# SahakyanLab/GenomeAssembler_dev

Hardware: AMD Instinct MI355X
Metric: k-mers built+scored/sec (higher is better)
Workload: dtype u64 keys / u32 counts / f64 scores; 1 GPU; cfg2 (configs[2]): 100 x 50000 bp segments per GPU, 150 bp reads at 50x, k=31, build + breakage scoring of all contigs; mode=segments, segments_total=100, distinct_kmers_rank0=3843627, parallelism=segments sharded over 1 GPU(s), no collective

## Files before the change

### genomeassembler_dev_amd/_lib.py

```python
import ctypes as C
import os

_HERE = os.path.dirname(os.path.abspath(__file__))
LIB_PATH = os.environ.get("GASM_LIBGASM") or os.path.join(_HERE, "libgasm.so")

GASM_OK = 0
STATUS = {0: "GASM_OK", -1: "GASM_ERR_INVALID", -2: "GASM_ERR_NON_ACGT", -3: "GASM_ERR_NO_DEVICE", -4: "GASM_ERR_HIP",
          -5: "GASM_ERR_CAPACITY", -6: "GASM_ERR_RANGE", -7: "GASM_ERR_STATE", -8: "GASM_ERR_INTERNAL"}
TABLE_ROWS = 69904
MAX_TIP_ROUNDS = 8
MAX_BUBBLE_ROUNDS = 8
MAX_BUBBLE_LEN = 65535
MAX_COV_ROUNDS = 8
CORRECT_FIELDS = ("no_kmer", "clean", "corrected", "partial", "left", "bases_changed")
CORRECT_MAX_KMERS = 4096
THREAD_MAX_KMERS = 4096
MAX_SPAN_LEN = 65535
MAX_INSERT = 65535
PAIR_FIELDS = ("skipped", "none_placed", "one_placed", "same_contig", "reversed", "diff_contig")
MAP_MAX_MISMATCH = 255
MAP_MAX_BLOCKS = 8
MAP_FIELDS = ("short", "skipped", "unseeded", "rejected", "mapped_one", "mapped_multi", "blocks_dropped")
MAP_MAX_GAP = 16
MAPG_FIELDS = MAP_FIELDS + ("gapped",)
# ... 19 lines not shown
_PP = C.POINTER(C.c_void_p)


class BuildParams(C.Structure):
    _fields_ = [("size", _u32), ("k", _i32), ("genome_len_hint", _u64), ("min_count", _u32), ("strands", _u32), ("tip_len", _u32),
                ("tip_rounds", _u32), ("bubble_len", _u32), ("bubble_rounds", _u32), ("cov_cutoff", _u32), ("cov_len", _u32), ("cov_rounds", _u32)]

    @classmethod
    def make(cls, k, **fields):
        p = cls(size=C.sizeof(cls), k=int(k))
        for name, v in fields.items():
            setattr(p, name, int(v))
        return p


SYMBOLS = {
    "gasm_last_error": (C.c_char_p, []),
    "gasm_version": (C.c_char_p, []),
    "gasm_ctx_create": (_int, [_int, _PP]),
    "gasm_ctx_destroy": (None, [_vp]),
    "gasm_ctx_sync": (_int, [_vp]),
    "gasm_ctx_stream": (_vp, [_vp]),
    "gasm_get_contigs": (_int, [_vp, _vp, _u64, _int, _int, _int, _PP]),
    "gasm_get_contigs_from_reads": (_int, [_vp, _vp, _vp, _u64, _int, _int, _int, _PP]),
    "gasm_get_contigs_from_reads_solid": (_int, [_vp, _vp, _vp, _u64, _int, _int, _int, _u32, _PP]),
    "gasm_get_contigs_from_reads_strands": (_int, [_vp, _vp, _vp, _u64, _int, _int, _int, _u32, _u32, _PP]),
    "gasm_get_contigs_from_reads_tips": (_int, [_vp, _vp, _vp, _u64, _int, _int, _int, _u32, _u32, _u32, _u32, _PP]),
    "gasm_get_contigs_from_reads_bubbles": (_int, [_vp, _vp, _vp, _u64, _int, _int, _int, _u32, _u32, _u32, _u32, _u32, _u32, _PP]),
    "gasm_get_contigs_from_reads_params": (_int, [_vp, _vp, _vp, _u64, _int, _int, C.POINTER(BuildParams), _PP]),
    "gasm_contigs_count": (_u64, [_vp]),
    "gasm_contigs_data": (_vp, [_vp]),
    "gasm_contigs_offsets": (_vp, [_vp]),
    "gasm_contigs_rows": (_u64, [_vp]),
    "gasm_contigs_perm": (_vp, [_vp]),
    "gasm_contigs_distinct_count": (_u64, [_vp]),
    "gasm_contigs_key_words": (_int, [_vp]),
    "gasm_contigs_distinct_keys": (_vp, [_vp]),
    "gasm_contigs_distinct_mult": (_vp, [_vp]),
    "gasm_contigs_free": (None, [_vp]),
    "gasm_assemble_contigs": (_int, [_vp, _vp, _vp, _u64, _vp, _u64, _u64, _int, _PP]),
    "gasm_assemble_contigs_velvet": (_int, [_vp, _vp, _vp, _u64, _int, _int, _int, _PP]),
    "gasm_assemble_contigs_dev": (_int, [_vp, _vp, _vp, _u64, _vp, _u64, _u64, _int, _PP]),
    "gasm_assemble_contigs_velvet_dev": (_int, [_vp, _vp, _vp, _u64, _int, _int, _int, _PP]),
    "gasm_scaffolds_count": (_u64, [_vp]),
    "gasm_scaffolds_offsets": (_vp, [_vp]),
    "gasm_scaffolds_merge_device": (_int, [_vp, C.POINTER(_u64)]),
    "gasm_scaffolds_fetch": (_int, [_vp, _PP]),
    "gasm_scaffolds_free": (None, [_vp]),
    "gasm_calc_breakscore_dev": (_int, [_vp, _vp, _vp, _vp, _u64, _vp, _u64, _int, _vp, _vp, _u64, _vp, _int, _int, _PP]),
    "gasm_strlist_count": (_u64, [_vp]),
    "gasm_strlist_data": (_vp, [_vp]),
    "gasm_strlist_offsets": (_vp, [_vp]),
    "gasm_strlist_free": (None, [_vp]),
    "gasm_calc_breakscore": (_int, [_vp, _vp, _vp, _u64, _vp, _vp, _u64, _vp, _u64, _int, _vp, _vp, _u64, _vp, _int, _int,
                                    _PP]),
    "gasm_calc_breakscore_tables": (_int, [_vp, _vp, _vp, _u64, _vp, _vp, _u64, _vp, _u64, _int, _vp, _vp, _u64, _vp, _u32, _int, _int, _PP]),
    "gasm_calc_breakscore_tables_dev": (_int, [_vp, _vp, _vp, _vp, _u64, _vp, _u64, _int, _vp, _vp, _u64, _vp, _u32, _int, _int, _PP]),
    "gasm_batch_score_tables": (_int, [_vp, _int, _vp, _u32]),
    "gasm_batch_fetch_scores_table": (_int, [_vp, _u32, _PP, _PP, _PP, _PP, _PP]),
    "gasm_batch_fetch_score_fixed_table": (_int, [_vp, _u32, _PP, C.POINTER(_int)]),
    "gasm_scores_count": (_u64, [_vp]),
    "gasm_scores_sequence_len": (_vp, [_vp]),
    "gasm_scores_bp_score": (_vp, [_vp]),
    "gasm_scores_norm_by_break_freqs": (_vp, [_vp]),
    "gasm_scores_norm_by_len": (_vp, [_vp]),
    "gasm_scores_kmer_breaks": (_vp, [_vp]),
    "gasm_scores_lev_dist": (_vp, [_vp]),
    "gasm_scores_path_freq": (_vp, [_vp]),
    "gasm_scores_startpos": (_vp, [_vp]),
    "gasm_scores_prob_dist": (_vp, [_vp]),
    "gasm_scores_prob_dist_offsets": (_vp, [_vp]),
    "gasm_scores_ks": (_vp, [_vp]),
    "gasm_scores_lev_device": (_int, [_vp]),
    "gasm_coverage_percent": (_int, [_vp, _vp, _vp, _u64, C.c_int64, _vp]),
    "gasm_scores_free": (None, [_vp]),
    "gasm_levenshtein": (_int, [_vp, _u64, _vp, _u64, _int, C.POINTER(_i32)]),
    "gasm_batch_create": (_int, [_vp, _vp, _vp, _u64, _u32, _vp, _u32, _PP]),
    "gasm_batch_create_packed": (_int, [_vp, _vp, _vp, _u64, _u32, _vp, _u32, _PP]),
    "gasm_batch_from_files": (_int, [_vp, _vp, _u32, _int, _PP, C.POINTER(_u64)]),
    "gasm_batch_guided": (_int, [_vp]),
    "gasm_batch_fetch_guided": (_int, [_vp, _PP, _PP, _PP, _PP, _PP, _PP]),
    "gasm_batch_fetch_score_fixed": (_int, [_vp, _PP, C.POINTER(_int)]),
    "gasm_batch_build_plan": (_int, [_vp, C.POINTER(_i32), _int]),
    "gasm_batch_simulate": (_int, [_vp, _vp, _vp, _u32, _u32, C.c_double, _u64, _int, _vp, _PP]),
    "gasm_batch_fetch_read_starts": (_int, [_vp, _PP, _PP]),
    "gasm_read_files": (_int, [_vp, _u32, _int, _PP]),
    "gasm_read_files_device": (_int, [_vp, _vp, _u32, _int, _PP]),
    "gasm_packed_parsed_on_device": (_int, [_vp, _u32]),
    "gasm_packed_n_reads": (_u64, [_vp]),
    "gasm_packed_n_segments": (_u32, [_vp]),
    "gasm_packed_words": (_vp, [_vp]),
    "gasm_packed_read_off": (_vp, [_vp]),
    "gasm_packed_seg_read_off": (_vp, [_vp]),
    "gasm_packed_dropped": (_u64, [_vp]),
    "gasm_packed_free": (None, [_vp]),
    "gasm_batch_free": (None, [_vp]),
    "gasm_batch_build": (_int, [_vp, _int, _u64]),
    "gasm_batch_score": (_int, [_vp, _int, _vp]),
    "gasm_batch_build_solid": (_int, [_vp, _int, _u64, _u32]),
    "gasm_batch_build_strands": (_int, [_vp, _int, _u64, _u32, _u32]),
    "gasm_batch_strands": (_u32, [_vp]),
    "gasm_batch_build_tips": (_int, [_vp, _int, _u64, _u32, _u32, _u32, _u32]),
    "gasm_batch_tip_len": (_u32, [_vp]),
    "gasm_batch_tip_rounds": (_u32, [_vp]),
    "gasm_batch_fetch_tip_stats": (_int, [_vp, _PP, _PP]),
    "gasm_batch_build_bubbles": (_int, [_vp, _int, _u64, _u32, _u32, _u32, _u32, _u32, _u32]),
    "gasm_batch_bubble_len": (_u32, [_vp]),
    "gasm_batch_bubble_rounds": (_u32, [_vp]),
    "gasm_batch_fetch_bubble_stats": (_int, [_vp, _PP, _PP]),
    "gasm_batch_build_params": (_int, [_vp, C.POINTER(BuildParams)]),
    "gasm_batch_cov_cutoff": (_u32, [_vp]),
    "gasm_batch_cov_len": (_u32, [_vp]),
    "gasm_batch_cov_rounds": (_u32, [_vp]),
    "gasm_batch_fetch_lowcov_stats": (_int, [_vp, _PP, _PP]),
    "gasm_batch_contig_coverage": (_int, [_vp]),
    "gasm_batch_fetch_contig_coverage": (_int, [_vp, _PP, _PP]),
    "gasm_batch_fetch_contig_twins": (_int, [_vp, _PP]),
    "gasm_batch_contig_links": (_int, [_vp, _u32]),
    "gasm_batch_fetch_contig_links": (_int, [_vp, _PP, _PP, _PP, _PP, _PP]),
    "gasm_batch_place_pairs": (_int, [_vp, _u32]),
    "gasm_batch_fetch_pair_places": (_int, [_vp, _PP, _PP, _PP, C.POINTER(_u32)]),
    "gasm_batch_map_reads": (_int, [_vp, _u32]),
    "gasm_batch_fetch_read_map": (_int, [_vp, _PP, _PP, _PP, _PP]),
    "gasm_batch_map_reads_gapped": (_int, [_vp, _u32, _u32]),
    "gasm_batch_fetch_read_map_gapped": (_int, [_vp, _PP, _PP, _PP, _PP, _PP, _PP]),
    "gasm_batch_map_reads_gapped_ends": (_int, [_vp, _u32, _u32, _u32]),
    "gasm_batch_fetch_read_map_ends": (_int, [_vp, _PP, _PP]),
    "gasm_batch_map_reads_aligned": (_int, [_vp, _u32, _u32, _u32]),
    "gasm_batch_fetch_read_alignments": (_int, [_vp, _PP, _PP, C.POINTER(_u32)]),
    "gasm_batch_score_mapped": (_int, [_vp, _int, _int, _vp, _u32, _u32]),
    "gasm_batch_fetch_mapped_scores": (_int, [_vp, _u32, _PP, _PP, _PP, _PP, _PP, _PP, C.POINTER(_int)]),
    "gasm_batch_fetch_mapped_starts": (_int, [_vp, _PP, _PP]),
    "gasm_batch_fetch_solid_stats": (_int, [_vp, _PP, _PP]),
    "gasm_batch_kmer_spectrum": (_int, [_vp]),
    "gasm_batch_fetch_kmer_spectrum": (_int, [_vp, _PP]),
    "gasm_batch_correct_reads": (_int, [_vp, _PP]),
    "gasm_batch_fetch_correct_stats": (_int, [_vp, _PP]),
    "gasm_batch_fetch_reads": (_int, [_vp, _PP, _PP]),
    "gasm_batch_total_kmers": (_u64, [_vp]),
    "gasm_batch_total_reads": (_u64, [_vp]),
    "gasm_batch_fetch_distinct": (_int, [_vp, _PP, _PP, _PP, C.POINTER(_int)]),
    "gasm_batch_fetch_contigs": (_int, [_vp, _PP, _PP, _PP]),
    "gasm_batch_fetch_graph": (_int, [_vp, _PP, _PP]),
    "gasm_batch_fetch_scores": (_int, [_vp, _PP, _PP, _PP, _PP, _PP]),
    "gasm_batch_count_read_kmers": (_int, [_vp]),
    "gasm_batch_fetch_read_kmer_counts": (_int, [_vp, _PP]),
    "gasm_count_read_kmers": (_int, [_vp, _vp, _vp, _u64, _int, _vp, _vp, _u64, _vp]),
    "gasm_pool_create": (_int, [_vp, _vp, _u64, _u32, _vp, _u32, _PP]),
    "gasm_pool_free": (None, [_vp]),
    "gasm_pool_key_words": (_int, [_vp]),
    "gasm_pool_local_runs": (_int, [_vp, _int, _int, _PP]),
    "gasm_pool_pack_runs": (_int, [_vp, _vp, _u64, _vp, _vp]),
    "gasm_pool_merge_runs": (_int, [_vp, _u32, _u32, _vp, _vp, _vp, _vp, _PP]),
    "gasm_pool_fetch_fine_directory": (_int, [_vp, _PP, C.POINTER(_int)]),
    "gasm_pool_graph": (_int, [_vp, _u32]),
    "gasm_pool_piece_words": (_int, [_vp, _u32, _u32, _vp]),
    "gasm_pool_pack_reads": (_int, [_vp, _u32, _u32, _vp]),
    "gasm_pool_set_reads": (_int, [_vp, _vp, _u64, _u32, _vp, _vp, _vp]),
    "gasm_pool_score": (_int, [_vp, _int, _vp]),
    "gasm_pool_fetch_distinct": (_int, [_vp, _PP, _PP, _PP, C.POINTER(_int)]),
    "gasm_pool_fetch_contigs": (_int, [_vp, _PP, _PP, _PP]),
    "gasm_pool_fetch_scores": (_int, [_vp, _PP, _PP, _PP, _PP, _PP]),
    "gasm_comm_unique_id": (_int, [_vp]),
    "gasm_comm_create": (_int, [_vp, _vp, _int, _int, _PP]),
    "gasm_comm_create_virtual": (_int, [_vp, _int, _PP]),
    "gasm_comm_destroy": (None, [_vp]),
# ... 117 lines not shown
```

### genomeassembler_dev_amd/batch.py

```python
import ctypes as C
from fractions import Fraction

import numpy as np

from . import qtable, readkmers
from ._lib import CORRECT_FIELDS, MAP_FIELDS, MAP_MAX_GAP, MAP_MAX_MISMATCH, MAP_MAX_PIECES, MAPEND_FIELDS, MAPG_FIELDS, MAPSCORE_FIELDS, MAPSCORE_PARTIAL, MAPSCORE_SOURCES, MAX_TABLES, MAX_BUBBLE_ROUNDS, MAX_COV_ROUNDS, MAX_INSERT, MAX_SPAN_LEN, MAX_TIP_ROUNDS, PAIR_FIELDS, PLAN_FIELDS, BuildParams, check, default_context, lib
from .api import _check_build_opts, unpack_kmers
from .links import ContigLinks
from .pairs import PairPlaces
from .readmap import AlignedReadMap, GappedReadMap, MappedScores, ReadMap


def _arr(p, ctype, n):
    return np.ctypeslib.as_array(C.cast(p, C.POINTER(ctype)), shape=(n,)).copy() if n else np.zeros(0, ctype)


def weighted_median_half(mult_sum, n_edges):
    ms, ns = [int(x) for x in mult_sum], [int(x) for x in n_edges]
    order = sorted(range(len(ns)), key=lambda i: Fraction(ms[i], ns[i]))
    total, run = sum(ns), 0
    for i in order:
        run += ns[i]
        if 2 * run >= total:
            return ms[i] // (2 * ns[i])
# ... 233 lines not shown
            check(lib().gasm_batch_fetch_read_map_ends(self.h, *[C.byref(p) for p in pe]))
            ends = dict(end_gap=end_gap, rec_end=_arr(pe[0], C.c_int32, 4 * self.n_reads), end_counters=_arr(pe[1], C.c_uint64, self.n_segments * len(MAPEND_FIELDS)))
        return GappedReadMap(self.k, strands, max_edits, max_gap, contigs, rec, gap, pile, gpile, hist, cnt,
                             [t.tolist() for t in self.contig_twins()] if strands == 2 else None, getattr(self, "_seg_read_off", None), **ends)

    def align_reads(self, max_edits=6, max_gap=3, end_gap=3):
        if not 0 <= int(max_edits) <= MAP_MAX_MISMATCH:
            raise ValueError(f"max_edits must be 0..{MAP_MAX_MISMATCH}")
        if not 0 <= int(max_gap) <= MAP_MAX_GAP:
            raise ValueError(f"max_gap must be 0..{MAP_MAX_GAP}")
        if not 0 <= int(end_gap) <= MAP_MAX_GAP:
            raise ValueError(f"end_gap must be 0..{MAP_MAX_GAP}")
        max_edits, max_gap, end_gap = int(max_edits), int(max_gap), int(end_gap)
        check(lib().gasm_batch_map_reads_aligned(self.h, max_edits, max_gap, end_gap))
        ps, pe, pa, cols = [C.c_void_p() for _ in range(6)], [C.c_void_p() for _ in range(2)], [C.c_void_p() for _ in range(2)], C.c_uint32()
        check(lib().gasm_batch_fetch_read_map_gapped(self.h, *[C.byref(p) for p in ps]))
        check(lib().gasm_batch_fetch_read_map_ends(self.h, *[C.byref(p) for p in pe]))
        check(lib().gasm_batch_fetch_read_alignments(self.h, *[C.byref(p) for p in pa], C.byref(cols)))
        seg, o, contigs = self._contigs_by_segment()
        total = int(o[-1]) if int(seg[-1]) else 0
        W = int(cols.value)
        rec, gap = _arr(ps[0], C.c_int32, 4 * self.n_reads), _arr(ps[1], C.c_int32, 4 * self.n_reads)
        pile, gpile = _arr(ps[2], C.c_uint32, 4 * total), _arr(ps[3], C.c_uint32, 2 * total)
        hist, cnt = _arr(ps[4], C.c_uint32, self.n_segments * (max_edits + 1)), _arr(ps[5], C.c_uint64, self.n_segments * len(MAPG_FIELDS))
        strands = self.strands()
        return AlignedReadMap(self.k, strands, max_edits, max_gap, end_gap, contigs, rec, gap, pile, gpile, hist, cnt,
                              _arr(pe[0], C.c_int32, 4 * self.n_reads), _arr(pe[1], C.c_uint64, self.n_segments * len(MAPEND_FIELDS)),
                              _arr(pa[0], C.c_int32, 2 * MAP_MAX_PIECES * self.n_reads), _arr(pa[1], C.c_uint32, 4 * W * total), W,
                              self._read_lengths(), [t.tolist() for t in self.contig_twins()] if strands == 2 else None,
                              getattr(self, "_seg_read_off", None))

    def score_mapped(self, kmer=8, tables=None, source="gapped", partial=False):
        t = np.ascontiguousarray(qtable.load_normalised() if tables is None else tables, dtype=np.float64)
        if t.ndim == 1:
            t = t.reshape(1, -1)
        if t.ndim != 2 or t.shape[1] != qtable.ROWS:
            raise ValueError(f"tables must be rows of {qtable.ROWS} probabilities")
        if not 1 <= t.shape[0] <= MAX_TABLES:
            raise ValueError(f"tables must hold 1..{MAX_TABLES} rows")
        if source not in MAPSCORE_SOURCES:
            raise ValueError(f"source must be one of {sorted(MAPSCORE_SOURCES)}")
        if int(kmer) < 0:
            raise ValueError("kmer must be >= 0")
        T = int(t.shape[0])
        check(lib().gasm_batch_score_mapped(self.h, MAPSCORE_SOURCES[source], int(kmer), t.ctypes.data_as(C.c_void_p), T, MAPSCORE_PARTIAL if partial else 0))
        seg, o, contigs = self._contigs_by_segment()
        n = int(seg[-1])
        total = int(o[-1]) if n else 0
        per_table = []
        for i in range(T):
            ps, sh = [C.c_void_p() for _ in range(6)], C.c_int()
            check(lib().gasm_batch_fetch_mapped_scores(self.h, i, *[C.byref(p) for p in ps], C.byref(sh)))
            per_table.append((dict(bp_score=_arr(ps[0], C.c_double, n), bp_score_norm_by_break_freqs=_arr(ps[1], C.c_double, n),
                                   bp_score_norm_by_len=_arr(ps[2], C.c_double, n), kmer_breaks=_arr(ps[3], C.c_int32, n),
                                   sequence_len=_arr(ps[4], C.c_int32, n), seg_contig_off=seg), _arr(ps[5], C.c_int64, n), sh.value))
        sp, cp = C.c_void_p(), C.c_void_p()
        check(lib().gasm_batch_fetch_mapped_starts(self.h, C.byref(sp), C.byref(cp)))
        return MappedScores(int(kmer), source, bool(partial), contigs, per_table, _arr(sp, C.c_uint32, total),
                            _arr(cp, C.c_uint64, self.n_segments * len(MAPSCORE_FIELDS)))

    def suggest_cov_cutoff(self, segment):
        floor = getattr(self, "_min_count", 1) + 1
        ms, ns = self.contig_coverage(segment)
        if not len(ns):
            return floor
        return max(floor, weighted_median_half(ms, ns))

    def kmer_spectrum(self):
        check(lib().gasm_batch_kmer_spectrum(self.h))
        p = C.c_void_p()
        check(lib().gasm_batch_fetch_kmer_spectrum(self.h, C.byref(p)))
        n = self.n_segments * 256
        return np.ctypeslib.as_array(C.cast(p, C.POINTER(C.c_uint64)), shape=(n,)).copy().reshape(self.n_segments, 256)

    def build_plan(self):
        rows = lib().gasm_batch_build_plan(self.h, None, 0)
        if rows < 0:
            check(rows)
        out = (C.c_int32 * (rows * len(PLAN_FIELDS)))()
        check(min(0, lib().gasm_batch_build_plan(self.h, out, len(out))))
        blocks = [dict(zip(PLAN_FIELDS, out[j * len(PLAN_FIELDS):(j + 1) * len(PLAN_FIELDS)])) for j in range(rows)]
        return dict(blocks[0], blocks=blocks)

    def score(self, kmer=8, table=None):
        t = np.ascontiguousarray(qtable.load_normalised() if table is None else table, dtype=np.float64)
        if t.size != qtable.ROWS:
            raise ValueError(f"table must hold {qtable.ROWS} probabilities")
        self._table = t
        check(lib().gasm_batch_score(self.h, int(kmer), t.ctypes.data_as(C.c_void_p)))
        return self

    def score_tables(self, kmer, tables):
        t = np.ascontiguousarray(tables, dtype=np.float64)
        if t.ndim != 2 or t.shape[1] != qtable.ROWS:
            raise ValueError(f"tables must be rows of {qtable.ROWS} probabilities")
        self._table = t[0] if len(t) else None
        check(lib().gasm_batch_score_tables(self.h, int(kmer), t.ctypes.data_as(C.c_void_p), t.shape[0]))
        return self

    def count_read_kmers(self):
        check(lib().gasm_batch_count_read_kmers(self.h))
        p = C.c_void_p()
        check(lib().gasm_batch_fetch_read_kmer_counts(self.h, C.byref(p)))
        n = self.n_segments * qtable.ROWS
        a = np.ctypeslib.as_array(C.cast(p, C.POINTER(C.c_uint32)), shape=(n,)).copy() if n else np.zeros(0, np.uint32)
        self._rkc = a.reshape(self.n_segments, qtable.ROWS)
        return self._rkc

    def read_kmer_counts(self, segment, kmer):
        if getattr(self, "_rkc", None) is None:
            self.count_read_kmers()
        return self._rkc[segment, readkmers.table_slice(kmer)]

    def correct_reads(self):
        h = C.c_void_p()
        check(lib().gasm_batch_correct_reads(self.h, C.byref(h)))
        new = SegmentBatch.__new__(SegmentBatch)
        new.ctx, new.h, new.k, new._table = self.ctx, h, None, None
        new.n_segments, new.n_reads = self.n_segments, int(lib().gasm_batch_total_reads(h))
        return new

    def correction_stats(self, as_dict=False):
        p = C.c_void_p()
        check(lib().gasm_batch_fetch_correct_stats(self.h, C.byref(p)))
        n = self.n_segments * len(CORRECT_FIELDS)
        a = np.ctypeslib.as_array(C.cast(p, C.POINTER(C.c_uint32)), shape=(n,)).copy().reshape(self.n_segments, len(CORRECT_FIELDS))
        return {name: a[:, i] for i, name in enumerate(CORRECT_FIELDS)} if as_dict else a

    def reads(self):
        d, o = C.c_void_p(), C.c_void_p()
        check(lib().gasm_batch_fetch_reads(self.h, C.byref(d), C.byref(o)))
        off = np.ctypeslib.as_array(C.cast(o, C.POINTER(C.c_uint64)), shape=(self.n_reads + 1,)).copy()
        total = int(off[-1])
        data = np.frombuffer(C.string_at(d, total), dtype=np.uint8).copy() if total else np.zeros(0, np.uint8)
        return data, off

    def read_strings(self):
        data, off = self.reads()
        raw = data.tobytes()
        return [raw[int(off[i]):int(off[i + 1])].decode() for i in range(self.n_reads)]

    def total_kmers(self):
        return int(lib().gasm_batch_total_kmers(self.h))

    def distinct(self):
        so, ks, ms, w = C.c_void_p(), C.c_void_p(), C.c_void_p(), C.c_int()
        check(lib().gasm_batch_fetch_distinct(self.h, C.byref(so), C.byref(ks), C.byref(ms), C.byref(w)))
        seg = np.ctypeslib.as_array(C.cast(so, C.POINTER(C.c_uint64)), shape=(self.n_segments + 1,)).copy()
        n = int(seg[-1])
        keys = np.ctypeslib.as_array(C.cast(ks, C.POINTER(C.c_uint64)), shape=(n * w.value,)).copy() if n else np.zeros(0, np.uint64)
        mult = np.ctypeslib.as_array(C.cast(ms, C.POINTER(C.c_uint32)), shape=(n,)).copy() if n else np.zeros(0, np.uint32)
        return seg, keys, mult, w.value

    def distinct_kmers(self, segment):
        seg, keys, mult, w = self.distinct()
        a, b = int(seg[segment]), int(seg[segment + 1])
        return unpack_kmers(keys[a * w:b * w], self.k, w), mult[a:b]

    def graph(self):
        seg = self.distinct()[0]
        n = int(seg[-1])
        fl, nx = C.c_void_p(), C.c_void_p()
        check(lib().gasm_batch_fetch_graph(self.h, C.byref(fl), C.byref(nx)))
        if not n:
            return np.zeros(0, np.uint8), np.zeros(0, np.uint32)
        return (np.ctypeslib.as_array(C.cast(fl, C.POINTER(C.c_uint8)), shape=(n,)).copy(),
# ... 74 lines not shown
```

### genomeassembler_dev_amd/csrc/capi.hip

```cpp
#include <algorithm>
#include <atomic>
#include <functional>
#include <memory>
#include <mutex>
#include <new>
#include <thread>

#include "pipeline.h"
#include "scaffolds.h"

struct gasm_strlist {
    std::vector<char> data;
    std::vector<u64> off;
};

struct gasm_contigs {
    std::vector<char> data;
    std::vector<u64> off;
    u64 rows = 0;
    std::vector<u32> perm;
    int words = 1;
    std::vector<u64> dkeys;
    std::vector<u32> dmult;
};
// ... 1166 lines not shown
    return GASM_OK;
}

int gasm_batch_score(gasm_batch* b, int kmer, const double* table) {
    API_GUARD_BEGIN
    return batch_score(b, "gasm_batch_score", kmer, table, 1);
    API_GUARD_END
}

int gasm_batch_score_tables(gasm_batch* b, int kmer, const double* tables, uint32_t n_tables) {
    API_GUARD_BEGIN
    return batch_score(b, "gasm_batch_score_tables", kmer, tables, n_tables);
    API_GUARD_END
}

int gasm_batch_guided(gasm_batch* b) {
    API_GUARD_BEGIN
    if (!b) { gasm_set_error("batch is null"); return GASM_ERR_INVALID; }
    if (!b->built || !b->scored) { gasm_set_error("gasm_batch_guided needs gasm_batch_build and gasm_batch_score first"); return GASM_ERR_STATE; }
    GCHK(batch_finish(b));
    StepSlot& x = b->S();
    GCHK(pipeline_score_fetch(x.cx, x.ss));
    return guided_build(x.cx, b->rd, x.bs, x.dp, x.ss, b->tb[0], b->score_kmer, b->guided);
    API_GUARD_END
}

int gasm_batch_fetch_guided(gasm_batch* b, const uint64_t** seg_off, const uint64_t** off, const char** data, const double** bp_score,
                            const double** norm_by_len, const int32_t** kmer_breaks) {
    API_GUARD_BEGIN
    if (!b || !seg_off || !off || !data || !bp_score || !norm_by_len || !kmer_breaks) { gasm_set_error("null argument"); return GASM_ERR_INVALID; }
    if (!b->guided.valid) { gasm_set_error("fetch before gasm_batch_guided"); return GASM_ERR_STATE; }
    GuidedState& g = b->guided;
    GCHK(guided_fetch_text(b->S().cx, g));
    *seg_off = g.h_seg_off.data(); *off = g.h_text_off.data(); *data = g.h_text.data();
    *bp_score = g.ss.h_bp.data(); *norm_by_len = g.ss.h_nl.data(); *kmer_breaks = g.ss.h_breaks.data();
    return GASM_OK;
    API_GUARD_END
}

static int batch_fetch_fixed(gasm_batch* b, uint32_t t, const int64_t** fx, int* shift) {
    if (!b || !fx || !shift) { gasm_set_error("null argument"); return GASM_ERR_INVALID; }
    if (!b->scored) { gasm_set_error("gasm_batch_fetch_score_fixed needs a scored batch"); return GASM_ERR_STATE; }
    if (t >= b->score_tables) { gasm_set_error("table %u of a score with %u table(s)", t, b->score_tables); return GASM_ERR_INVALID; }
    GCHK(batch_finish(b));
    StepSlot& x = b->S();
    if (!x.ss.graph) {
        gasm_set_error("the batch was scored in FP64, not in fixed point (reads shorter than k, or a table with NaN / infinite entries or a "
                       "range the 64-bit fixed point cannot hold): there are no fixed-point sums");
        return GASM_ERR_STATE;
    }
    const u32 P = x.bs.n_contigs;
    b->h_fx.resize(P);
    const size_t fx_off = (x.ss.stride * 4 + 15) & ~(size_t)15;
    HIPCHK(hipSetDevice(b->ctx->device));
    if (P) HIPCHK(hipMemcpyAsync(b->h_fx.data(), static_cast<const char*>(x.ss.d_total.p) + fx_off + (size_t)t * x.ss.stride * 8, (size_t)P * 8, hipMemcpyDeviceToHost, x.cx->stream));
    HIPCHK(hipStreamSynchronize(x.cx->stream));
    *fx = b->h_fx.data();
    *shift = b->tb[t].fix_shift;
    return GASM_OK;
}

int gasm_batch_fetch_score_fixed(gasm_batch* b, const int64_t** fx, int* shift) {
    API_GUARD_BEGIN
    return batch_fetch_fixed(b, 0, fx, shift);
    API_GUARD_END
}

int gasm_batch_fetch_score_fixed_table(gasm_batch* b, uint32_t t, const int64_t** fx, int* shift) {
    API_GUARD_BEGIN
    return batch_fetch_fixed(b, t, fx, shift);
    API_GUARD_END
}

int gasm_batch_build_plan(gasm_batch* b, int32_t* out, int n) {
    API_GUARD_BEGIN
    if (!b || n < 0 || (n > 0 && !out)) { gasm_set_error("gasm_batch_build_plan: bad argument"); return GASM_ERR_INVALID; }
    if (!b->built) { gasm_set_error("gasm_batch_build_plan before gasm_batch_build"); return GASM_ERR_STATE; }
    GCHK(batch_finish(b));
    if (n >= GASM_PLAN_FIELDS) pipeline_build_plan(b->rd, b->S().bs, out);
    return 1;
    API_GUARD_END
}

int gasm_batch_count_read_kmers(gasm_batch* b) {
    API_GUARD_BEGIN
    if (!b) { gasm_set_error("batch is null"); return GASM_ERR_INVALID; }
    if (!b->rkc_checked) GCHK(read_kmer_windows_check(b->rd));
    b->rkc_checked = true;
    HIPCHK(hipSetDevice(b->ctx->device));
    GCHK(b->d_rkc.ensure((size_t)b->n_segments * GASM_TABLE_ROWS * 4));
    GCHK(launch_read_kmer_count(b->ctx, b->rd, b->d_rkc.as<u32>()));
    b->rkc_counted = true;
    return GASM_OK;
    API_GUARD_END
}

int gasm_batch_fetch_read_kmer_counts(gasm_batch* b, const uint32_t** counts) {
    API_GUARD_BEGIN
    if (!b || !counts) { gasm_set_error("gasm_batch_fetch_read_kmer_counts: null argument"); return GASM_ERR_INVALID; }
    if (!b->rkc_counted) { gasm_set_error("gasm_batch_fetch_read_kmer_counts before gasm_batch_count_read_kmers"); return GASM_ERR_STATE; }
    b->h_rkc.resize((size_t)b->n_segments * GASM_TABLE_ROWS);
    HIPCHK(hipSetDevice(b->ctx->device));
    HIPCHK(hipMemcpyAsync(b->h_rkc.data(), b->d_rkc.p, b->h_rkc.size() * 4, hipMemcpyDeviceToHost, b->ctx->stream));
    HIPCHK(hipStreamSynchronize(b->ctx->stream));
    *counts = b->h_rkc.data();
    return GASM_OK;
    API_GUARD_END
}

int gasm_batch_correct_reads(gasm_batch* b, gasm_batch** out) {
    API_GUARD_BEGIN
    if (!b || !out) { gasm_set_error("gasm_batch_correct_reads: null argument"); return GASM_ERR_INVALID; }
    *out = nullptr;
    if (!b->built) { gasm_set_error("gasm_batch_correct_reads before a build"); return GASM_ERR_STATE; }
    GCHK(batch_finish(b));
    StepSlot& x = b->S();
    DBuf words, stats;
    struct Rel { DBuf &a, &b; ~Rel() { a.release(); b.release(); } } rel{words, stats};
    GCHK(pipeline_correct_reads(x.cx, b->rd, x.bs, words, stats));
    HIPCHK(hipStreamSynchronize(x.cx->stream));
    const DevReads& rd = b->rd;
    return new_batch(b->ctx, b->n_segments, rd.n_reads, out, [&](gasm_batch* nb) {
        GCHK(nb->rd.adopt_packed(b->ctx, words, rd.fixed_len ? nullptr : rd.h_read_off.data(), rd.n_reads, rd.fixed_len, rd.h_seg_read_off.data(), rd.n_segments));
        std::swap(nb->d_correct, stats);
        nb->corrected = true;
        return (int)GASM_OK;
    });
    API_GUARD_END
}

int gasm_batch_fetch_correct_stats(gasm_batch* b, const uint32_t** stats) {
    API_GUARD_BEGIN
    if (!b || !stats) { gasm_set_error("gasm_batch_fetch_correct_stats: null argument"); return GASM_ERR_INVALID; }
    if (!b->corrected) { gasm_set_error("gasm_batch_fetch_correct_stats: not a batch made by gasm_batch_correct_reads"); return GASM_ERR_STATE; }
    b->h_correct.resize((size_t)b->n_segments * GASM_CORRECT_FIELDS);
    HIPCHK(hipSetDevice(b->ctx->device));
    HIPCHK(hipMemcpyAsync(b->h_correct.data(), b->d_correct.p, b->h_correct.size() * 4, hipMemcpyDeviceToHost, b->ctx->stream));
    HIPCHK(hipStreamSynchronize(b->ctx->stream));
    *stats = b->h_correct.data();
    return GASM_OK;
    API_GUARD_END
}

int gasm_batch_fetch_reads(gasm_batch* b, const char** ascii, const uint64_t** read_off) {
    API_GUARD_BEGIN
    if (!b || !ascii || !read_off) { gasm_set_error("gasm_batch_fetch_reads: null argument"); return GASM_ERR_INVALID; }
    GCHK(pipeline_fetch_reads(b->ctx, b->rd, b->h_reads_ascii, b->h_reads_off));
    *ascii = b->h_reads_ascii.data();
    *read_off = b->h_reads_off.data();
    return GASM_OK;
    API_GUARD_END
}

static const u32 kRkcRow[9] = {0, 0, 0, 0, 16, 0, 272, 0, 4368};

int gasm_count_read_kmers(gasm_ctx* ctx, const char* reads, const uint64_t* read_off, uint64_t n_reads, int kmer, const char* keys,
                          const uint64_t* key_off, uint64_t n_keys, uint32_t* counts) {
    API_GUARD_BEGIN
    if (!ctx || (n_reads && (!reads || !read_off)) || (keys && n_keys && !key_off)) { gasm_set_error("gasm_count_read_kmers: null argument"); return GASM_ERR_INVALID; }
    if (kmer != 2 && kmer != 4 && kmer != 6 && kmer != 8) { gasm_set_error("kmer must be 2, 4, 6 or 8 (got %d)", kmer); return GASM_ERR_INVALID; }
    const u64 n_out = keys ? n_keys : (1ull << (2 * kmer));
    if (n_out && !counts) { gasm_set_error("gasm_count_read_kmers: counts is null"); return GASM_ERR_INVALID; }
    std::vector<u32> row;
    if (keys) {
        row.resize(n_keys);
        for (u64 i = 0; i < n_keys; ++i) {
// ... 105 lines not shown
```

### genomeassembler_dev_amd/csrc/kernels.h

```cpp
#pragma once
#include <hip/hip_runtime.h>
#include <stdint.h>

#include <type_traits>

#include "device_utils.h"
#include "keyops.h"

struct ReadSet {
    const u64* words;
    const u64* read_off;
    const u64* seg_read_off;
    const u32* seg_tile_start;
    const uint4* tile_info;
    u32 fixed_len;
    u32 n_segments;
};

__device__ __forceinline__ void read_span(const ReadSet& rs, u64 r, u64* p0, u32* len) {
    if (rs.fixed_len) { *p0 = rs.read_off ? rs.read_off[r] : r * rs.fixed_len; *len = rs.fixed_len; }
    else { const u64 a = rs.read_off[r]; *p0 = a; *len = (u32)(rs.read_off[r + 1] - a); }
}

struct GraphView {
    const void* dk_key;
    const u32* dstart;
    const u16* fdir;
    int k;
    int bbits;
    int fbits;
};

template <class K>
__device__ __forceinline__ u32 graph_lower_bound(const GraphView& gv, u32 seg, const K& t, u32* bucket_hi) {
    const K* dk = reinterpret_cast<const K*>(gv.dk_key);
    const u32 nb = 1u << gv.bbits;
    const int low = 2 * gv.k - gv.bbits;
    const u32 gb = seg * nb + (gv.bbits ? kfield(t, low) : 0u);
    uint2 dd;
    __builtin_memcpy(&dd, gv.dstart + gb, 8);
    const u32 base = dd.x;
    *bucket_hi = dd.y;
    const int bshift = low > gv.fbits ? low - gv.fbits : 0;
    const u32 nbin = 1u << gv.fbits;
    const u16* f = gv.fdir + (u64)gb * (nbin + 1) + (kfield(t, bshift) & (nbin - 1));
    u32 ff;
    __builtin_memcpy(&ff, f, 4);
    u32 lo = base + (ff & 0xFFFFu);
    u32 hi = base + (ff >> 16);
    if (hi > *bucket_hi) hi = *bucket_hi;
    if (lo > hi) lo = hi;
    while (hi - lo > 4) {
        const u32 m = (lo + hi) >> 1;
        if (kless(dk[m], t)) lo = m + 1;
        else hi = m;
    }
    while (lo < hi && kless(dk[lo], t)) ++lo;
    return lo;
}

struct PathSet {
    const u64* words;
    const u64* p_off;
    const u32* seg_path_off;
    u32 n_segments;
};

#define GASM_KT 16
#define GASM_SCORE_PATH_CAP 6144
#define GASM_TBL 4096
#define GASM_TBL_LIMIT 2816
constexpr int dedup_bins(int tbl) { return tbl / 4; }
constexpr int dedup_fbits(int tbl) { return tbl <= 4 ? 0 : 1 + dedup_fbits(tbl / 2); }
static_assert(1 << dedup_fbits(2048) == dedup_bins(2048) && 1 << dedup_fbits(GASM_TBL) == dedup_bins(GASM_TBL), "the bins are a power of two");

enum : u32 {
    GASM_FLAG_OVERFLOW = 0,
    GASM_FLAG_RANK_FAILED = 1,
    GASM_FLAG_SCORE_MISMATCH = 2,
    GASM_FLAG_DEDUP_DONE = 8,
    GASM_FLAG_CONTIG_DONE = 9,
    GASM_FLAG_SOLID_DONE = 10,
    GASM_FLAG_ACTIVE = 16,
    GASM_FLAG_ACTIVE_N = 40,
    GASM_FLAG_WORDS = 64,
    GASM_FLAG_CURSORS = 64,
    GASM_FLAG_BYTES = 256,
    GASM_OVF_TABLE = 1,
    GASM_OVF_REGION = 2,
    GASM_OVF_TIP_RANK = 4,
};
static_assert(GASM_FLAG_ACTIVE + GASM_FLAG_ACTIVE_N <= GASM_FLAG_WORDS && GASM_FLAG_WORDS * 4 == GASM_FLAG_BYTES, "flag area layout");

template <class W>
struct BuildReport {
    W* w;
    u32 S;
    __host__ __device__ W& dstart(u32 s) const { return w[s]; }
    __host__ __device__ W& cstart(u32 s) const { return (w + S + 1)[s]; }
    __host__ __device__ W& bstart_lo(u32 s) const { return (w + 2 * S + 2)[2 * s]; }
    __host__ __device__ W& bstart_hi(u32 s) const { return (w + 2 * S + 2)[2 * s + 1]; }
    __host__ __device__ W& flags() const { return w[4 * S + 4]; }
    __host__ __device__ W& rank_failed() const { return w[4 * S + 5]; }
    __host__ __device__ W& ticket() const { return w[4 * S + 6]; }
    static size_t words(u32 S) { return 4 * (size_t)S + 8; }
};

__global__ void k_pack_ascii(const u8* ascii, u64 nbases_host, const u64* nbases_dev, u64* words, u32* err);
#define GASM_TILE_WG 512
template <class K> struct TileStage {
    static constexpr u32 KPU = 16 / sizeof(K);
    static constexpr u32 CAP = KeyTraits<K>::NFL * GASM_TILE_WG * KPU;
    static constexpr u32 TRASH = GASM_TILE_WG / 8;
    static constexpr u32 BYTES = (CAP + TRASH) * (u32)sizeof(K);
    static constexpr u32 PAD_ROOM = (KeyTraits<K>::NFL * KPU - KeyTraits<K>::KT) * GASM_TILE_WG;
};
template <class K> struct ScatterLds {
    u32 nb;
    static constexpr u32 n_key = TileStage<K>::CAP + TileStage<K>::TRASH;
    constexpr u32 n_comb() const { return (nb + 1) & ~1u; }
    constexpr u32 n_sub() const { return 4 * nb; }
    static constexpr u32 n_dummy = 4;
    static constexpr u32 n_tmp = 12;
    constexpr size_t total() const { return TileStage<K>::BYTES + (size_t)nb * 8 + ((size_t)n_sub() + n_dummy + n_tmp) * 4 + 32; }
};
template <class K> struct PartitionLds {
    u32 nb;
    static constexpr u32 n_key = TileStage<K>::CAP + TileStage<K>::TRASH;
    constexpr u32 n_comb() const { return nb; }
    constexpr u32 n_sub() const { return 4 * nb; }
    static constexpr u32 n_dummy = 4;
    static constexpr u32 n_tmp = 12;
    constexpr u32 n_cin() const { return nb; }
    constexpr size_t total() const { return TileStage<K>::BYTES + (size_t)n_comb() * 16 + (2 * ((size_t)n_sub() + n_dummy) + n_tmp + n_cin()) * 4; }
};
#define GASM_FLUSH_WGS 1024
#define GASM_FLUSH_SLOTS (GASM_FLUSH_WGS * (GASM_TILE_WG / 64))
__device__ __forceinline__ u32 flush_slot(u32 wave) { return (blockIdx.x % GASM_FLUSH_WGS) * (GASM_TILE_WG / 64) + wave; }
template <class K> __global__ void k_tile_hist(ReadSet rs, const uint4* tinfo, int k, int bbits, u32 g, u32 n_tiles, ushort4* tcnt);
__global__ void k_tile_scan(ReadSet rs, int bbits, u32 padm, const ushort4* tcnt, u32* toff, u32* hist, u32* flags);
template <class TO> __global__ void k_scan_excl(const u32* in, TO* out, u32 n);
__global__ void k_copy_u64(const u64* a, u64* b, u32 n);
template <class K>
__global__ void k_bucket_scatter(ReadSet rs, const uint4* tinfo, int k, int bbits, u32 g, u32 padm, u32 n_tiles, const u64* bstart, const u32* toff,
                                 const ushort4* tcnt, K* keys, u64 scratch);
#define GASM_RT_MAX 16
template <class K>
__global__ void k_bucket_partition(ReadSet rs, const uint4* tinfo, int k, int bbits, u32 g, u32 padm, u32 n_tiles, const u64* bstart, u32* cursor,
                                   K* keys, u64 scratch, u32* flags);
template <class K, int TBL>
__global__ void k_bucket_dedup(K* keys, u32* mult, const u64* bstart, const u32* blen, u32* bucket_d, u32* overflow, u16* fdir, int low_bits, u32* dstart);
#define GASM_BUCKET_MAX 65535
template <class K>
__global__ void k_bucket_dedup_multi(const K* keys, K* keys_out, u32* mult, const u64* bstart, u32* bucket_d, u32* overflow, u16* fdir, int low_bits);
template <class K>
__global__ void k_bucket_solid(K* keys, u32* mult, const u64* bstart, u32* bucket_d, u16* fdir, int low_bits, int fbits, int bbits, u32 min_count,
                               u32* removed, u32* done, u32* dstart);
template <class K>
__global__ void k_tip_mark(GraphView gv, u32 n_segments, u32 chunks, const u8* eflag, const u32* clen, const u32* nxt, const u32* dk_cnt, const u64* bstart,
                           u32* mult, u32 tip_len, u32* flags, u32* tips);
template <class K>
__global__ void k_bubble_mark(GraphView gv, u32 n_segments, u32 chunks, const u8* eflag, const u32* clen, const u32* nxt, const u32* dk_cnt, const u64* bstart,
                              u32* mult, u32 bubble_len, u32* flags, u32* bubbles);
__global__ void k_kmer_spectrum(const u32* dstart, u32 nb, const u32* dk_cnt, u32 n_segments, u32 chunks, u32* hist);
template <class K>
__global__ void k_lowcov_mark(GraphView gv, u32 n_segments, u32 chunks, const u8* eflag, const u32* clen, const u32* nxt, const u32* dk_cnt, const u64* bstart,
                              u32* mult, u32 cov_len, u32 cov_cutoff, u32* flags, u32* removed);
__global__ void k_contig_cov(const u32* dstart, u32 nb, u32 n_segments, u32 chunks, const u64* link, const u32* e_cid, const u32* dk_cnt,
                             const u32* seg_cstart, unsigned long long* msum, u32* nedges);
template <class K>
__global__ void k_bucket_gather(const K* keys, const u32* mult, const u64* bstart, const u32* dstart, K* dk_key, u32* dk_cnt, u32* claim, u8* eflag,
                                u32* flags);
template <class K> __global__ void k_edge_target(GraphView gv, u32 n_segments, u32 chunks, u32* tgt, u32* claim);
__global__ void k_edge_multi(GraphView gv, u32 n_segments, u32 chunks, const u32* tgt, const u32* claim, u8* eflag);
template <class K>
__global__ void k_node_flags(GraphView gv, u32 n_segments, u32 chunks, const u32* claim, u8* eflag, u64* link, u32* clen);
__global__ void k_edge_next(GraphView gv, u32 n_segments, u32 chunks, const u32* tgt, const u8* eflag, u32* nxt, u64* link);
__global__ void k_link_jump(GraphView gv, u32 n_segments, u32 chunks, u64* link, const u32* prev_active, u32* active, int jumps, const u32* nxt,
                            u32* clen);
__global__ void k_rank_rulers(GraphView gv, u32 n_segments, u32 chunks, u64* link, u32* rtab, u32 rshift, u32* flags);
__global__ void k_rank_lds(GraphView gv, const u32* rtab, u64* link, int max_rounds, u32 rshift, u32 lds_entries, u32* flags);
__global__ void k_chain_len(const u32* nxt, const u64* link, u32* clen, const u32* n_edges_p);
__global__ void k_contig_scan(GraphView gv, const u8* eflag, const u32* clen, u32* e_cid, u64* e_coff, u32* seg_ncontig,
                              u64* seg_cbases, u32* done, u32* seg_cstart, u64* seg_bstart, const u32* flags, u32* report, u32 ticket);
__global__ void k_contig_place(GraphView gv, const u8* eflag, const u32* seg_cstart, const u64* seg_bstart, u32* e_cid, u64* e_coff,
                               u64* c_off, u32 n_segments, u32 chunks);
template <class K>
__global__ void k_contig_emit(GraphView gv, const u64* link, const u32* nxt, const u64* e_coff, u8* out, u32 n_segments, u32 chunks);
__global__ void k_reads_both_strands(const u64* words, const u64* read_off, const u64* seg_read_off, u32 fixed_len, u32 n_segments, u64 n_reads, u32 g,
                                     unsigned long long* out);
template <class K>
__global__ void k_contig_twin(GraphView gv, const u64* link, const u32* e_cid, const u64* c_off, const u32* seg_cstart, const u8* text, u32 n_segments,
                              u32* twin, u32* bad);

template <class K>
__global__ void k_pack_runs(const K* keys, const u32* mult, const u64* bstart, const u32* bucket_d, const u32* gb_list, const u64* dst_off, K* out_keys,
                            u32* out_cnt);
template <class K, int TBL>
__global__ void k_bucket_merge(const K* in_keys, const u32* in_cnt, const u64* run_off, const u32* run_len, u32 n_src, K* out_keys, u32* out_cnt,
                               const u64* bstart, u32* bucket_d, u32* overflow, u16* fdir, int low_bits, const u64* src_base);
__global__ void k_repack_reads(const u64* src, const u64* dir, u64* words_out);
__global__ void k_piece_positions(const u64* piece_first, const u64* piece_word_off, u32 n_pieces, u64 n_reads, u32 fixed_len, u64* pos);
__global__ void k_slice_last(const u32* a, const u64* off, u32 n, u32* out);

__global__ void k_chain_expand(const u64* cwords, const u64* c_off, const u64* sig_off, const u32* elem_contig, const u32* elem_skip, const u64* elem_pos,
                               const u64* out_off, u32 n_scaffolds, u64* out, u64 n_words);
struct ChainSigs {
    const u64* sig_off;
    const u32* elem_contig;
    const u32* elem_skip;
    const u64* elem_pos;
};
__global__ void k_str_bitonic(const u64* words, const u64* off, u32* idx, u32 n_pow2, u32 kk, u32 j, ChainSigs cs);
__global__ void k_str_bitonic_block(const u64* words, const u64* off, u32* idx, u32 n_pow2, u32 kk, u32 j0, ChainSigs cs);
__global__ void k_str_adjacent_eq(const u64* words, const u64* off, const u32* idx, u32 n, u8* same_as_prev, ChainSigs cs);
__global__ void k_unpack_ascii(const u64* words, u64 nbases, u8* out);
__global__ void k_guided_chain(PathSet ps, const unsigned long long* fx, int k, u32* g_next, u32* g_prev, u32* dbg_order);
__global__ void k_asm_match(const u64* cwords, const u64* c_off, u32 n, int k, u8* match, u8* row_any, u8* level_any);
__global__ void k_asm_merge(const u32* perm, u32 rows, u32 n, int k, const u32* clen, const u8* match, const u8* row_any, const u8* level_any,
                            const u64* cwords, const u64* c_off, u32* out_next, u8* out_ov, u32* out_heads, u32* out_nchains, u8* need_host);

__global__ void k_sim_weights(const u64* gwords, const u64* gbase, const u64* woff, u32 n_segments, int kmer, const long long* fixw, u64* w);
template <class T> __global__ void k_seg_scan_incl(T* a, const u64* off);
__global__ void k_sim_draw(const u64* cum, const u64* woff, const u64* doff, const u64* glen, u64 seed, u32 read_len, u32* start, u32* keep);
__global__ void k_sim_compact(const u32* start, const u32* keep, const u32* rank, const u64* doff, const u64* seg_read_off, u32* kept_start);
__global__ void k_sim_extract(const u64* gwords, const u64* gbase, const u64* seg_read_off, const u32* kept_start, u32 read_len, unsigned long long* out);

template <int LS>
__global__ void k_read_kmer_count(const u64* words, const u64* read_off, const u64* seg_read_off, u32 fixed_len, u32 n_segments, u32* out);

struct ContigIndex {
    const u64* link;
// ... 106 lines not shown
```

### genomeassembler_dev_amd/csrc/kernels_build.hip

```cpp
#include "device_utils.h"
#include "keyops.h"
#include "kernels.h"
#include "dedup_order.h"

typedef unsigned long long u64x2 __attribute__((ext_vector_type(2)));

typedef unsigned int u32x4nt __attribute__((ext_vector_type(4)));
__device__ __forceinline__ uint4 stream_load16(const uint4* p) {
    const u32x4nt v = __builtin_nontemporal_load(reinterpret_cast<const u32x4nt*>(p));
    return make_uint4(v.x, v.y, v.z, v.w);
}
__device__ __forceinline__ void stream_store16(u64x2 v, u64x2* p) { __builtin_nontemporal_store(v, p); }

__global__ void __launch_bounds__(GASM_WG) k_pack_ascii(const u8* __restrict__ ascii, u64 nbases_host, const u64* __restrict__ nbases_dev,
                                                        u64* __restrict__ words, u32* __restrict__ err) {
    const u64 nbases = nbases_dev ? *nbases_dev : nbases_host;
    const u64 nwords = (nbases + 31) / 32 + 4;
    bool ok = true;
    for (u64 t = (u64)blockIdx.x * GASM_WG + threadIdx.x; t < nwords; t += (u64)gridDim.x * GASM_WG) {
        const u64 b0 = t << 5;
        u64 w = 0;
        if (b0 + 32 <= nbases) {
            const uint4* src = reinterpret_cast<const uint4*>(ascii + b0);
            const uint4 v0 = src[0], v1 = src[1];
// ... 231 lines not shown
            pf.bs_lo = b.x; pf.bs_hi = b.y;
        }
        tile_fetch<K>(rs, ti, g, k, pf.rl, pf.nv);
    };
    TileInfo ti = tile_decode(tinfo, tile);
    TilePrefetch<K> pf;
    fetch(tile, ti, pf);
    pf.template wait_all_but<0>();
    for (;;) {
        u32 total;
        if (one) {
            const u32 c0 = pf.c01 & 0xFFFFu, c1 = pf.c01 >> 16, c2 = pf.c23 & 0xFFFFu, c3 = pf.c23 >> 16;
            const u32 cnt = c0 + c1 + c2 + c3, padc = (cnt + padm) & ~padm;
            const u32 soff = block_excl_scan<GASM_TILE_WG>(padc, s_tmp, &total);
            if (tid < nb) {
                *reinterpret_cast<uint4*>(&s_cur[4 * tid]) = make_uint4(soff, soff + c0, soff + c0 + c1, soff + c0 + c1 + c2);
                s_comb[tid] = (((u64)pf.bs_hi << 32) | pf.bs_lo) + pf.toff - soff;
                for (u32 i = cnt; i < padc; ++i) s_key[soff + i] = key_filler<K>(tid, bshift);
            }
        } else {
            u32 carry = 0;
            for (u32 b0 = 0; b0 < nb; b0 += GASM_TILE_WG) {
                const u32 b = b0 + tid;
                const ushort4 c = tcnt[(u64)tile * nb + b];
                const u32 cnt = sub_total(c), padc = (cnt + padm) & ~padm;
                u32 tot;
                const u32 soff = carry + block_excl_scan<GASM_TILE_WG>(padc, s_tmp, &tot);
                *reinterpret_cast<uint4*>(&s_cur[4 * b]) = make_uint4(soff, soff + c.x, soff + c.x + c.y, soff + c.x + c.y + c.z);
                s_comb[b] = bstart[(u64)ti.seg * nb + b] + toff[(u64)tile * nb + b] - soff;
                for (u32 i = cnt; i < padc; ++i) s_key[soff + i] = key_filler<K>(b, bshift);
                carry += tot;
            }
            total = carry;
        }
        __syncthreads();
        const auto w = pf.rl.prep();
        const u32 nv = pf.nv;
        K key[KT];
        u32 idx[KT];
        static_for<KT>([&](auto J) {
            constexpr u32 j = J;
            key[j] = w.template key<j>(k);
            const u32 bkt = bbits ? w.template top_hi<j>() >> (32 - bbits) : 0u;
            idx[j] = atomicAdd(&s_cur[j < nv ? 4 * bkt + sub : 4 * nb], 1u);
        });
        const u32 tnext = tile + 1 < tile_end ? tile + 1 : tile;
        const TileInfo tin = tile_decode(tinfo, tnext);
        fetch(tnext, tin, pf);
        const u32 trash = CAP + wv * 8 + (ln & 7u);
#pragma unroll
        for (u32 j = 0; j < KT; ++j) s_key[j < nv ? idx[j] : trash] = key[j];
        __syncthreads();
        static_assert(NFL % 3 == 0, "flush passes come in threes");
#pragma unroll
        for (u32 u0 = 0; u0 < NFL; u0 += 3) {
            u64x2 w[3];
            u64 cb[3];
#pragma unroll
            for (u32 u = 0; u < 3; ++u) w[u] = *reinterpret_cast<const u64x2*>(s_key + (tid + GASM_TILE_WG * (u0 + u)) * KPU);
#pragma unroll
            for (u32 u = 0; u < 3; ++u) {
                u32 bkt = 0;
                if (bbits) {
                    if constexpr (KPU == 2) bkt = (u32)(w[u].x >> bshift) & (nb - 1);
                    else bkt = kfield(K128{w[u].x, w[u].y}, bshift) & (nb - 1);
                }
                cb[u] = s_comb[bkt];
            }
#pragma unroll
            for (u32 u = 0; u < 3; ++u) {
                const u32 i = (tid + GASM_TILE_WG * (u0 + u)) * KPU;
                stream_store16(w[u], reinterpret_cast<u64x2*>(keys + (i < total ? cb[u] + i : my_scratch)));
            }
        }
        if (++tile >= tile_end) break;
        __syncthreads();
        ti = tin;
        pf.template wait_all_but<NFL>();
    }
}
template __global__ void k_bucket_scatter<u64>(ReadSet, const uint4*, int, int, u32, u32, u32, const u64*, const u32*, const ushort4*, u64*, u64);
template __global__ void k_bucket_scatter<K128>(ReadSet, const uint4*, int, int, u32, u32, u32, const u64*, const u32*, const ushort4*, K128*, u64);

template <class K>
__global__ void __launch_bounds__(GASM_TILE_WG, 4) k_bucket_partition(ReadSet rs, const uint4* __restrict__ tinfo, int k, int bbits, u32 g, u32 padm,
                                                                    u32 n_tiles, const u64* __restrict__ bstart, u32* __restrict__ cursor,
                                                                    K* __restrict__ keys, u64 scratch, u32* __restrict__ flags) {
    extern __shared__ __align__(16) unsigned char s_raw[];
    constexpr u32 KT = KeyTraits<K>::KT;
    constexpr u32 NFL = KeyTraits<K>::NFL;
    constexpr u32 KPU = TileStage<K>::KPU;
    constexpr u32 CAP = TileStage<K>::CAP;
    const u32 nb = 1u << bbits;
    const u32 tid = threadIdx.x, wv = tid >> 6, ln = tid & 63, sub = tid & 3u;
    const PartitionLds<K> lds{nb};
    K* s_key = reinterpret_cast<K*>(s_raw);
    uint4* s_comb = reinterpret_cast<uint4*>(s_key + lds.n_key);
    u32* s_base = reinterpret_cast<u32*>(s_comb + lds.n_comb());
    u32* s_cnt = s_base + lds.n_sub() + lds.n_dummy;
    u32* s_tmp = s_cnt + lds.n_sub() + lds.n_dummy;
    u32* s_cin = s_tmp + lds.n_tmp;
    const int bshift = 2 * k - bbits;
    const bool carry = padm != 0;
    const u32 ush = carry ? (u32)__builtin_ctz(padm + 1) - (KPU == 2 ? 1u : 0u) : 0u;
    const u32 n_carry = carry ? nb << ush : 0u;
    const u32 unit_m = carry ? KPU - 1 : 0u;

    const u32 per_wg = (n_tiles + gridDim.x - 1) / gridDim.x;
    const u32 tile_end = min(n_tiles, (blockIdx.x + 1) * per_wg);
    u32 tile = blockIdx.x * per_wg;
    if (tile >= tile_end) return;
    for (u32 e = tid; e < 4 * nb + 4; e += GASM_TILE_WG) s_cnt[e] = 0;

    Roll<K> rl;
    u32 nv;
    auto fetch = [&](const TileInfo& t) { tile_fetch<K>(rs, t, g, k, rl, nv); };
    TileInfo ti = tile_decode(tinfo, tile);
    fetch(ti);
    rl.template wait_all_but<0>();
    __syncthreads();
    bool fresh = true;
    u64x2 cu = {0, 0};
    for (;;) {
        const auto w = rl.prep();
        const u32 nv_now = nv;
        const u32 seg = ti.seg;
        u32 idx[KT];
        static_for<KT>([&](auto J) {
            constexpr u32 j = J;
            const u32 bkt = bbits ? w.template top_hi<j>() >> (32 - bbits) : 0u;
            idx[j] = atomicAdd(&s_cnt[j < nv_now ? 4 * bkt + sub : 4 * nb], 1u);
        });
        const u32 tnext = tile + 1 < tile_end ? tile + 1 : tile;
        const TileInfo tin = tile_decode(tinfo, tnext);
        fetch(tin);
        const bool last = !carry || tile + 1 >= tile_end || tin.seg != seg;
        __syncthreads();
        u32 t = tid, zero = 0;
        __asm__ volatile("" : "+v"(t), "+v"(zero));
        u32 c0 = 0, c1 = 0, c2 = 0, c3 = 0, cin = 0;
        if (t < nb) {
            const uint4 c = *reinterpret_cast<const uint4*>(&s_cnt[4 * t]);
            c0 = c.x; c1 = c.y; c2 = c.z; c3 = c.w;
            if (!fresh) cin = s_comb[t].w & 31u;
        }
        const u32 cnt = cin + c0 + c1 + c2 + c3, flush = cnt & ~padm;
        const u32 res = last ? (cnt + padm) & ~padm : flush;
        u32 total;
        const u32 both = block_excl_scan_open<GASM_TILE_WG>((((cnt + padm) & ~padm) << 16) | ((cnt + unit_m) & ~unit_m), s_tmp, &total);
        const bool lines = (total >> 16) <= CAP;
        const u32 soff = lines ? both >> 16 : both & 0xFFFFu;
        u32 run = 0;
        u64 beg = 0, end = 0;
        if (t < nb) {
            const u32 gb = seg * nb + t;
            if (res) run = atomicAdd(&cursor[gb], res);
            beg = bstart[gb]; end = bstart[gb + 1];
            const u32 s0 = soff + cin;
            *reinterpret_cast<uint4*>(&s_base[4 * t]) = make_uint4(s0, s0 + c0, s0 + c0 + c1, s0 + c0 + c1 + c2);
            *reinterpret_cast<uint4*>(&s_cnt[4 * t]) = make_uint4(zero, zero, zero, zero);
            s_cin[t] = (soff << 5) | cin;
            s_comb[t].w = (lines ? 1u << 31 : 0u) | ((soff + flush) << 5) | (cnt - flush);
        }
        __syncthreads();
        if (t < n_carry) {
            const u32 b = t >> ush, f = (t & ((1u << ush) - 1u)) * KPU;
            if (!fresh) {
                const u32 v = s_cin[b], n = v & 31u;
                K* const dst = s_key + (v >> 5) + f;
                if constexpr (KPU == 2) {
                    if (f < n) dst[0] = cu.x;
                    if (f + 1 < n) dst[1] = cu.y;
                } else {
                    if (f < n) *reinterpret_cast<u64x2*>(dst) = cu;
                }
            }
            const u32 v = s_comb[b].w, n = v & 31u;
            if ((v >> 31) && n) {
                K* const dst = s_key + ((v << 1) >> 6) + f;
                if (f >= n) dst[0] = key_filler<K>(b, bshift);
                if constexpr (KPU == 2) if (f + 1 >= n) dst[1] = key_filler<K>(b, bshift);
            }
        }
        {
            static_for<KT>([&](auto J) {
                constexpr u32 j = J;
                const u32 bkt = bbits ? w.template top_hi<j>() >> (32 - bbits) : 0u;
                idx[j] += s_base[4 * bkt + sub];
            });
            const u32 trash = CAP + wv * 8 + (ln & 7u);
            static_for<KT>([&](auto J) {
                constexpr u32 j = J;
                s_key[j < nv_now ? idx[j] : trash] = w.template key<j>(k);
            });
        }
        if (t < nb) {
            const bool fits = (u64)run + res <= end - beg;
            const u64 cb = beg + run - soff;
            s_comb[t] = make_uint4((u32)cb, (u32)(cb >> 32), fits ? soff + flush : 1u << 31, (lines ? 1u << 31 : 0u) | ((soff + flush) << 5) | (cnt - flush));
            if (!fits) atomicOr(flags + GASM_FLAG_OVERFLOW, GASM_OVF_REGION);
        }
        __syncthreads();
        if (t < n_carry) {
            const u32 b = t >> ush, f = (t & ((1u << ush) - 1u)) * KPU;
            const uint4 c = s_comb[b];
            const u32 rbeg = (c.w << 1) >> 6, n = c.w & 31u;
            cu = *reinterpret_cast<const u64x2*>(s_key + rbeg + f);
            if (last && n && !(c.z >> 31)) {
                u64x2 o = cu;
                if constexpr (KPU == 2) {
                    const u64 fl = key_filler<u64>(b, bshift);
                    if (f >= n) o.x = fl;
                    if (f + 1 >= n) o.y = fl;
                } else if (f >= n) {
                    const K128 fl = key_filler<K128>(b, bshift);
                    o.x = fl.hi; o.y = fl.lo;
                }
                stream_store16(o, reinterpret_cast<u64x2*>(keys + ((((u64)c.y << 32) | c.x) + rbeg + f)));
            }
        }
        const u64 my_scratch = scratch + (u64)flush_slot(t >> 6) * KPU;
        static_assert(NFL % 3 == 0, "flush passes come in threes");
#pragma unroll
        for (u32 u0 = 0; u0 < NFL; u0 += 3) {
            u64x2 wd[3];
            uint4 cb[3];
#pragma unroll
            for (u32 u = 0; u < 3; ++u) wd[u] = *reinterpret_cast<const u64x2*>(s_key + (t + GASM_TILE_WG * (u0 + u)) * KPU);
#pragma unroll
            for (u32 u = 0; u < 3; ++u) {
                u32 bkt = 0;
                if (bbits) {
                    if constexpr (KPU == 2) bkt = (u32)(wd[u].x >> bshift) & (nb - 1);
                    else bkt = kfield(K128{wd[u].x, wd[u].y}, bshift) & (nb - 1);
                }
                cb[u] = s_comb[bkt];
            }
#pragma unroll
            for (u32 u = 0; u < 3; ++u) {
                const u32 i = (t + GASM_TILE_WG * (u0 + u)) * KPU;
                stream_store16(wd[u], reinterpret_cast<u64x2*>(keys + ((int)i < (int)cb[u].z ? (((u64)cb[u].y << 32) | cb[u].x) + i : my_scratch)));
            }
        }
        if (++tile >= tile_end) break;
        ti = tin;
        fresh = last;
        rl.template wait_all_but<NFL>();
    }
}
template __global__ void k_bucket_partition<u64>(ReadSet, const uint4*, int, int, u32, u32, u32, const u64*, u32*, u64*, u64, u32*);
template __global__ void k_bucket_partition<K128>(ReadSet, const uint4*, int, int, u32, u32, u32, const u64*, u32*, K128*, u64, u32*);

#define GASM_SLOT_LOCKED 0xFFFFFFFFu

__device__ __forceinline__ u64x2 lds_load128(const void* p) {
    __asm__ volatile("" ::: "memory");
    return *reinterpret_cast<const u64x2*>(p);
}
__device__ __forceinline__ uint4 lds_load128u(const void* p) {
    __asm__ volatile("" ::: "memory");
    return *reinterpret_cast<const uint4*>(p);
}

template <int TBL>
__device__ __forceinline__ bool dedup_step(u64* t_key, u32* t_cnt, u32* n_distinct, u64 key, u32& set) {
    constexpr u32 NSETS = TBL / 2;
    const u64x2 c = lds_load128(&t_key[2 * set]);
    int slot = c.x == key ? 0 : c.y == key ? 1 : -1;
    if (slot < 0) {
        const int emp = c.x == GASM_EMPTY64 ? 0 : c.y == GASM_EMPTY64 ? 1 : -1;
        if (emp < 0) { set = (set + 1) & (NSETS - 1); return false; }
        const u64 old = atomicCAS(reinterpret_cast<unsigned long long*>(&t_key[2 * set + emp]), (unsigned long long)GASM_EMPTY64,
                                  (unsigned long long)key);
        if (old == GASM_EMPTY64) atomicAdd(n_distinct, 1u);
        else if (old != key) return false;
        slot = emp;
    }
    atomicAdd(&t_cnt[2 * set + slot], 1u);
    return true;
}
template <int TBL>
__device__ __forceinline__ bool dedup_step(K128* t_key, u32* t_cnt, u32* n_distinct, const K128& key, u32& set) {
    constexpr u32 NSETS = TBL / 2;
    __asm__ volatile("" ::: "memory");
    const uint2 c = *reinterpret_cast<const uint2*>(&t_cnt[2 * set]);
    const u32 cc[2] = {c.x, c.y};
#pragma unroll
    for (int q = 0; q < 2; ++q) {
        if (cc[q] == GASM_SLOT_LOCKED) return false;
        if (cc[q] == 0) {
            if (atomicCAS(&t_cnt[2 * set + q], 0u, GASM_SLOT_LOCKED) != 0u) return false;
            t_key[2 * set + q] = key;
            __builtin_amdgcn_fence(__ATOMIC_RELEASE, "workgroup");
            __hip_atomic_store(&t_cnt[2 * set + q], 1u, __ATOMIC_RELAXED, __HIP_MEMORY_SCOPE_WORKGROUP);
            atomicAdd(n_distinct, 1u);
            return true;
        }
        const u64x2 kq = lds_load128(&t_key[2 * set + q]);
        if (kq.x == key.hi && kq.y == key.lo) { atomicAdd(&t_cnt[2 * set + q], 1u); return true; }
    }
    set = set + 1 >= NSETS - 1 ? 0u : set + 1;
    return false;
}

constexpr int GASM_DEDUP_NLD = 3, GASM_DEDUP_NLDW = 6, GASM_DEDUP_WGS = 6;
__device__ __forceinline__ void publish_u32(u32* p, u32 v) { __hip_atomic_store(p, v, __ATOMIC_RELAXED, __HIP_MEMORY_SCOPE_AGENT); }
__device__ __forceinline__ void publish_u64(u64* p, u64 v) { __hip_atomic_store(p, v, __ATOMIC_RELAXED, __HIP_MEMORY_SCOPE_AGENT); }
__device__ __forceinline__ bool count_in_last(u32* done) {
    __asm__ volatile("s_waitcnt vmcnt(0)" ::: "memory");
    return __hip_atomic_fetch_add(done, 1u, __ATOMIC_RELAXED, __HIP_MEMORY_SCOPE_AGENT) == gridDim.x - 1;
}

__device__ __forceinline__ void dedup_last_scan(const u32* __restrict__ bucket_d, u32* __restrict__ dstart, u32 n, u32* __restrict__ done, u32* s_word,
                                                u32* s_waves ) {
    if (!dstart) return;
    __syncthreads();
    if (threadIdx.x == 0) *s_word = count_in_last(done) ? 1u : 0u;
    __syncthreads();
    if (!*s_word) return;
    const u32 per = (n + GASM_WG - 1) / GASM_WG, a = min(n, threadIdx.x * per), b = min(n, a + per);
    u32 sum = 0;
    for (u32 i = a; i < b; ++i) sum += __hip_atomic_load(&bucket_d[i], __ATOMIC_RELAXED, __HIP_MEMORY_SCOPE_AGENT);
    const u32 inc = wave_incl_scan(sum);
    __syncthreads();
    if ((threadIdx.x & 63) == 63) s_waves[threadIdx.x >> 6] = inc;
    __syncthreads();
    u32 ex = inc - sum, tot = 0;
    for (u32 w = 0; w < GASM_WG / 64; ++w) { const u32 t = s_waves[w]; if (w < (threadIdx.x >> 6)) ex += t; tot += t; }
    for (u32 i = a; i < b; ++i) { dstart[i] = ex; ex += __hip_atomic_load(&bucket_d[i], __ATOMIC_RELAXED, __HIP_MEMORY_SCOPE_AGENT); }
    if (threadIdx.x == 0) dstart[n] = tot;
}

template <class K, int TBL>
__global__ void __launch_bounds__(GASM_WG, TBL == 4096 ? 3 : sizeof(K) == 8 ? GASM_DEDUP_WGS : 4)
k_bucket_dedup(K* __restrict__ keys, u32* __restrict__ mult, const u64* __restrict__ bstart, const u32* __restrict__ blen, u32* __restrict__ bucket_d,
               u32* __restrict__ overflow, u16* __restrict__ fdir, int low_bits, u32* __restrict__ dstart) {
    constexpr int LIMIT = TBL / 16 * 11;
    constexpr int BINS = dedup_bins(TBL);
    constexpr int LOG_TBL = TBL == 4096 ? 12 : 11;
    constexpr bool WIDE = sizeof(K) == 16;
    constexpr int LOG_SETS = LOG_TBL - 1;
    constexpr u32 NSETS = 1u << LOG_SETS;
    static_assert(TBL == 4096 || TBL == 2048, "table size");
    __shared__ __align__(32) K t_key[TBL];
    __shared__ __align__(16) u32 t_cnt[TBL];
    u32 *s_tmp, *w_distinct, *w_overflow;
    if constexpr (WIDE) {
        s_tmp = reinterpret_cast<u32*>(&t_key[TBL - 2]);
        w_distinct = &t_cnt[TBL - 2];
        w_overflow = &t_cnt[TBL - 1];
    } else {
        __shared__ u32 s_tmp_narrow[8];
        s_tmp = s_tmp_narrow;
        w_distinct = &s_tmp_narrow[4];
        w_overflow = &s_tmp_narrow[5];
    }
    static_assert((TBL - LIMIT) * sizeof(K) >= 2 * BINS * sizeof(u32), "the bins must fit behind the sorted entries");
    u32* const s_start = reinterpret_cast<u32*>(t_key + LIMIT);
    u32* const s_cur = s_start + BINS;
    const u32 bucket = blockIdx.x;
    const u64 beg = bstart[bucket], end = bstart[bucket + 1];
// ... 36 lines not shown
            u32 missed = 0, mfull = 0;
            {
                u32 set[KPL];
                u64x2 c[KPL];
#pragma unroll
                for (int q = 0; q < KPL; ++q) {
                    set[q] = khash(kx[q]) >> (32 - LOG_SETS);
                    c[q] = lds_load128(&t_key[2 * set[q]]);
                }
#pragma unroll
                for (int q = 0; q < KPL; ++q) {
                    const u64 key = kx[q];
                    if (kis_filler(key)) continue;
                    const int slot = c[q].x == key ? 0 : c[q].y == key ? 1 : -1;
                    if (slot >= 0) atomicAdd(&t_cnt[2 * set[q] + slot], 1u);
                    else {
                        missed |= 1u << q;
                        if (c[q].y != GASM_EMPTY64) mfull |= 1u << q;
                    }
                }
            }
            while (missed) {
                const u32 q = (u32)__builtin_ctz(missed);
                missed &= missed - 1;
                u64 key = kx[0];
#pragma unroll
                for (u32 e = 1; e < (u32)KPL; ++e) if (e == q) key = kx[e];
                u32 st = ((khash(key) >> (32 - LOG_SETS)) + (mfull >> q & 1u)) & (NSETS - 1);
                bool ok = false;
                for (u32 probe = 0; probe < 8 * NSETS && !ok; ++probe) ok = dedup_step<TBL>(t_key, t_cnt, w_distinct, key, st);
                if (!ok) *w_overflow = 1;
            }
        } else {
            u32 set[KPL];
            uint2 cn[KPL];
            u64x2 k0[KPL], k1[KPL];
#pragma unroll
            for (int q = 0; q < KPL; ++q) {
                set[q] = min(khash(kx[q]) >> (32 - LOG_SETS), NSETS - 2);
                __asm__ volatile("" ::: "memory");
                cn[q] = *reinterpret_cast<const uint2*>(&t_cnt[2 * set[q]]);
                k0[q] = lds_load128(&t_key[2 * set[q]]);
                k1[q] = lds_load128(&t_key[2 * set[q] + 1]);
            }
            u32 missed = 0;
#pragma unroll
            for (int q = 0; q < KPL; ++q) {
                const K128 key = kx[q];
                if (kis_filler(key)) continue;
                const bool r0 = cn[q].x != 0 && cn[q].x != GASM_SLOT_LOCKED, r1 = cn[q].y != 0 && cn[q].y != GASM_SLOT_LOCKED;
                if (r0 && k0[q].x == key.hi && k0[q].y == key.lo) atomicAdd(&t_cnt[2 * set[q]], 1u);
                else if (r0 && r1 && k1[q].x == key.hi && k1[q].y == key.lo) atomicAdd(&t_cnt[2 * set[q] + 1], 1u);
                else missed |= 1u << q;
            }
            while (missed) {
                const u32 q = (u32)__builtin_ctz(missed);
                missed &= missed - 1;
                K128 key = kx[0];
#pragma unroll
                for (u32 e = 1; e < (u32)KPL; ++e) if (e == q) key = kx[e];
                u32 st = min(khash(key) >> (32 - LOG_SETS), NSETS - 2);
                bool ok = false;
                for (u32 probe = 0; probe < 8 * NSETS && !ok; ++probe) ok = dedup_step<TBL>(t_key, t_cnt, w_distinct, key, st);
                if (!ok) *w_overflow = 1;
            }
        }
    }
    __syncthreads();
    if (*w_overflow || *w_distinct > (u32)LIMIT) {
        for (u32 i = threadIdx.x; i <= (u32)BINS; i += GASM_WG) fdir[(u64)bucket * (BINS + 1) + i] = 0;
        if (threadIdx.x == 0) { atomicOr(overflow + GASM_FLAG_OVERFLOW, GASM_OVF_TABLE); publish_u32(&bucket_d[bucket], 0u); }
        dedup_last_scan(bucket_d, dstart, gridDim.x, overflow + GASM_FLAG_DEDUP_DONE, s_tmp + 7, s_tmp);
        return;
    }
    const u32 d = *w_distinct;
    dedup_order<K, TBL, true>(t_key, t_cnt, s_start, s_cur, s_tmp, fdir, bucket, low_bits, d);
    for (u32 i = threadIdx.x; i < d; i += GASM_WG) { keys[beg + i] = t_key[i]; mult[beg + i] = t_cnt[i]; }
    if (threadIdx.x == 0) publish_u32(&bucket_d[bucket], d);
    dedup_last_scan(bucket_d, dstart, gridDim.x, overflow + GASM_FLAG_DEDUP_DONE, s_tmp + 7, s_tmp);
}
template __global__ void k_bucket_dedup<u64, 4096>(u64*, u32*, const u64*, const u32*, u32*, u32*, u16*, int, u32*);
template __global__ void k_bucket_dedup<u64, 2048>(u64*, u32*, const u64*, const u32*, u32*, u32*, u16*, int, u32*);
template __global__ void k_bucket_dedup<K128, 2048>(K128*, u32*, const u64*, const u32*, u32*, u32*, u16*, int, u32*);

template <class K>
__global__ void __launch_bounds__(GASM_WG) k_bucket_dedup_multi(const K* __restrict__ keys, K* __restrict__ keys_out, u32* __restrict__ mult,
                                                                const u64* __restrict__ bstart, u32* __restrict__ bucket_d,
                                                                u32* __restrict__ overflow, u16* __restrict__ fdir, int low_bits) {
    constexpr int TBL = 4096, LIMIT = TBL / 16 * 11, BINS = dedup_bins(TBL), LOG_SETS = 11, LOG_BINS = dedup_fbits(TBL);
    constexpr u32 NSETS = 1u << LOG_SETS;
    __shared__ __align__(32) K t_key[TBL];
    __shared__ __align__(16) u32 t_cnt[TBL];
    __shared__ u32 s_start[BINS];
    __shared__ u32 s_cur[BINS];
    __shared__ u32 s_tmp[8];
    const u32 bucket = blockIdx.x;
    const u64 beg = bstart[bucket], n = bstart[bucket + 1] - beg;
    const int bin_bits = low_bits < LOG_BINS ? low_bits : LOG_BINS;
    const int r_max = low_bits < 16 ? low_bits : 16;
    u16* const fd = fdir + (u64)bucket * (BINS + 1);
    auto give_up = [&]() {
        for (u32 i = threadIdx.x; i <= (u32)BINS; i += GASM_WG) fd[i] = 0;
        if (threadIdx.x == 0) { atomicOr(overflow + GASM_FLAG_OVERFLOW, GASM_OVF_TABLE); bucket_d[bucket] = 0; }
    };
    for (int r = 0;; ++r) {
        if (r > r_max) { give_up(); return; }
        const u32 npass = 1u << r;
        u32 total = 0;
        bool fits = true;
        for (u32 p = 0; p < npass; ++p) {
            for (u32 i = threadIdx.x; i < TBL; i += GASM_WG) { t_key[i] = key_empty<K>(); t_cnt[i] = 0; }
            for (u32 i = threadIdx.x; i < BINS; i += GASM_WG) s_start[i] = 0;
            if (threadIdx.x == 0) { s_tmp[4] = 0; s_tmp[5] = 0; s_tmp[6] = 0; }
            __syncthreads();
            for (u64 i = threadIdx.x; i < n; i += GASM_WG) {
                const K key = keys[beg + i];
                if (kis_filler(key)) continue;
                if (r && (kfield(key, low_bits - r) & (npass - 1)) != p) continue;
                if (__hip_atomic_load(&s_tmp[4], __ATOMIC_RELAXED, __HIP_MEMORY_SCOPE_WORKGROUP) > (u32)LIMIT) break;
                u32 st = khash(key) >> (32 - LOG_SETS);
                bool ok = false;
                for (u32 probe = 0; probe < 8 * NSETS && !ok; ++probe) ok = dedup_step<TBL>(t_key, t_cnt, &s_tmp[4], key, st);
                if (!ok) s_tmp[5] = 1;
            }
            __syncthreads();
            const u32 d = s_tmp[4];
            if (s_tmp[5] || d > (u32)LIMIT) { fits = false; break; }
            if (total + d > GASM_BUCKET_MAX) { give_up(); return; }
            u32 lo, hi;
            if (r <= bin_bits) { lo = p << (bin_bits - r); hi = (p + 1) << (bin_bits - r); }
            else { lo = p >> (r - bin_bits); hi = (p & ((1u << (r - bin_bits)) - 1u)) ? lo : lo + 1; }
            dedup_order<K, TBL, false, true>(t_key, t_cnt, s_start, s_cur, s_tmp, fdir, bucket, low_bits, d, total, lo, hi);
            for (u32 i = threadIdx.x; i < d; i += GASM_WG) { keys_out[beg + total + i] = t_key[i]; mult[beg + total + i] = t_cnt[i]; }
            total += d;
            __syncthreads();
        }
        if (!fits) { __syncthreads(); continue; }
        for (u32 i = (1u << bin_bits) + threadIdx.x; i <= (u32)BINS; i += GASM_WG) fd[i] = (u16)total;
        if (threadIdx.x == 0) bucket_d[bucket] = total;
        return;
    }
}
template __global__ void k_bucket_dedup_multi<u64>(const u64*, u64*, u32*, const u64*, u32*, u32*, u16*, int);
template __global__ void k_bucket_dedup_multi<K128>(const K128*, K128*, u32*, const u64*, u32*, u32*, u16*, int);

#define GASM_SOLID_ITEMS 4
template <class K>
__global__ void __launch_bounds__(GASM_WG) k_bucket_solid(K* __restrict__ keys, u32* __restrict__ mult, const u64* __restrict__ bstart,
                                                          u32* __restrict__ bucket_d, u16* __restrict__ fdir, int low_bits, int fbits, int bbits,
                                                          u32 min_count, u32* __restrict__ removed, u32* __restrict__ done, u32* __restrict__ dstart) {
    constexpr u32 MAX_BINS = dedup_bins(GASM_TBL);
    constexpr u32 CHUNK = GASM_WG * GASM_SOLID_ITEMS;
    __shared__ u32 s_bin[MAX_BINS];
    __shared__ u32 s_tmp[8];
    const u32 bucket = blockIdx.x;
    const u32 bins = 1u << fbits;
    const int bshift = low_bits > fbits ? low_bits - fbits : 0;
    const u64 beg = bstart[bucket];
    const u32 d = bucket_d[bucket];
    for (u32 i = threadIdx.x; i < bins; i += GASM_WG) s_bin[i] = 0;
    __syncthreads();
    u32 out = 0;
    for (u32 base = 0; base < d; base += CHUNK) {
        K rk[GASM_SOLID_ITEMS];
        u32 rc[GASM_SOLID_ITEMS];
        u32 n_keep = 0;
// ... 724 lines not shown
```

### genomeassembler_dev_amd/csrc/pipeline.h

```cpp
#pragma once
#include "gasm_internal.h"
#include "kernels.h"

template <class K> struct KeyTag { using type = K; };
template <class F> static inline int with_key(int words, F&& f) { return words == 1 ? f(KeyTag<u64>{}) : f(KeyTag<K128>{}); }
#define GLAUNCH_K(ctx, words, name, kern, grid, block, shmem, ...)          \
    GCHK(with_key(words, [&](auto _tag) -> int {                            \
        using K = typename decltype(_tag)::type;                            \
        GLAUNCH(ctx, name, kern, grid, block, shmem, __VA_ARGS__);          \
        return GASM_OK;                                                     \
    }))

struct DevReads {
    u32 n_segments = 0;
    u64 n_reads = 0, total_bases = 0;
    u32 fixed_len = 0;
    u32 min_len = 0, max_len = 0;
    u64 n_empty = 0;
    std::vector<u64> h_read_off;
    std::vector<u64> h_seg_read_off;
    std::vector<u64> h_seg_empty;
    bool positioned = false;
    int sim_shift = 52;
    u64 upload_id = 0;
// ... 18 lines not shown
    u64 read_len(u64 r) const { return fixed_len ? fixed_len : h_read_off[r + 1] - h_read_off[r]; }
    void release();
};

struct DevPaths {
    u32 n_segments = 0, n_paths = 0;
    u64 total_bases = 0;
    std::vector<u64> h_p_off;
    std::vector<u32> h_seg_path_off;
    std::vector<u64> h_seg_base_off;
    DBuf d_words, d_p_off, d_seg_path_off, d_seg_base_off;
    const u64* b_p_off = nullptr;
    const u32* b_seg_path_off = nullptr;
    const u64* b_seg_base_off = nullptr;
    const u64* seg_base_off_dev() const { return b_seg_base_off ? b_seg_base_off : d_seg_base_off.as<u64>(); }
    int pack_from_device_ascii(gasm_ctx* ctx, const u8* d_ascii);
    int upload_ascii(gasm_ctx* ctx, const char* data, const u64* off, u32 n_paths);
    int upload_dirs(gasm_ctx* ctx);
    PathSet view() const;
    void release();
};

enum RoundKind : u32 { ROUNDS_TIP = 0, ROUNDS_BUBBLE, ROUNDS_LOWCOV, ROUND_KINDS };
struct BuildOpts {
    int k = 0;
    u64 genome_len_hint = 0;
    u32 min_count = 1, strands = 1, tip_len = 0, tip_rounds = 0, bubble_len = 0, bubble_rounds = 0, cov_cutoff = 0, cov_len = 0, cov_rounds = 0;
    bool lowcov() const { return cov_cutoff != 0 && cov_len != 0; }
    u32 rounds(u32 kind) const { return kind == ROUNDS_TIP ? tip_rounds : kind == ROUNDS_BUBBLE ? bubble_rounds : cov_rounds; }
    u32 total_rounds() const { return tip_rounds + bubble_rounds + cov_rounds; }
};
int build_opts_check(const BuildOpts& o);
BuildOpts build_opts_normalised(BuildOpts o);

struct RoundStats {
    u32 max_rounds;
    DBuf d_stats;
    std::vector<u32> h_contigs, h_kmers;
};

struct PassTable {
    size_t n, elem, align;
    bool zeroed;
    size_t off = 0;
    size_t bytes() const { return n * elem; }
};
struct PassLayout {
    std::vector<PassTable> t;
    size_t bytes = 0, zero_from = 0;
    PassLayout(std::initializer_list<PassTable> tables) : t(tables) {
        bool z = false;
        for (PassTable& x : t) {
            x.off = (bytes + x.align - 1) / x.align * x.align;
            if (x.zeroed && !z) { z = true; zero_from = x.off; }
            bytes = x.off + x.bytes();
        }
        if (!z) zero_from = bytes;
    }
    template <class T> T* at(const DBuf& d, size_t i) const { return reinterpret_cast<T*>(static_cast<char*>(d.p) + t[i].off); }
};
struct PassState {
    DBuf d;
    std::vector<std::vector<u64>> h;
    bool queued = false;
    u32 param[2] = {0, 0};
    template <class T> const T* host(size_t i) const { return reinterpret_cast<const T*>(h[i].data()); }
};
enum { LINKS_SUCC, LINKS_PRED, LINKS_LSUP, LINKS_SSUP, LINKS_SKIPPED };
enum { PAIRS_REC, PAIRS_HIST, PAIRS_CNT };
enum { MAP_REC, MAP_PILE, MAP_HIST, MAP_CNT };
enum { MAPG_REC, MAPG_GAP, MAPG_PILE, MAPG_GPILE, MAPG_HIST, MAPG_CNT, MAPG_END, MAPG_ENDCNT, MAPG_PIECE, MAPG_INS };
enum : u32 { MAPG_HAS_ENDS = 1u, MAPG_HAS_TRACE = 2u, MAPG_COLS_SHIFT = 8u };
enum { MAPSC_F64, MAPSC_I32, MAPSC_CNT, MAPSC_FX, MAPSC_PILE, MAPSC_COUNTERS };

struct BuildState {
    int k = 0, bbits = 0, fbits = 9, words = 1, bb_cap = 0;
    bool small_tbl = true;
    bool rank_global = false;
    bool single_pass = true;
    struct PartLayout {
        u64 reads_id = 0;
        int k = 0, bbits = 0, slack = 0, forced = 0;
        u32 padm = 0, g = 0;
        bool operator==(const PartLayout& o) const {
            return reads_id == o.reads_id && k == o.k && bbits == o.bbits && slack == o.slack && forced == o.forced && padm == o.padm && g == o.g;
        }
    } part;
    bool part_valid = false;
    u64 part_alloc = 0;
    bool multi_pass = false;
    bool ranked_in_lds = false;
    u32 tile_g = 1;
    u64 n_kmers = 0, hint = 0, reads_id = 0;
    BuildOpts opts;
    std::vector<u64> h_seg_nk;
    u64 D_cap = 0, maxD_cap = 0, bases_cap = 0;
    u32 maxD_est = 1, paths_est = 0;
    bool have_actual = false;
    u32 tile_orr = 1;
    bool part_single = false;
    bool scan_in_dedup = false;
    u32 ruler_shift = 0;
    u32 attempts_distinct = 0;
    u32 attempts_graph = 0;
    u32* h_report = nullptr;
    size_t h_report_words = 0;
    u32 ticket = 0;
    bool pending = false;
    u32 d_total = 0, n_contigs = 0;
    u64 contig_bases = 0;
    std::vector<u32> h_dstart;
    std::vector<u32> h_seg_cstart;
    std::vector<u64> h_seg_bstart;
    DBuf d_keys2;
    DBuf d_keys, d_mult, d_hist, d_toff, d_tcnt, d_fdir, d_bstart, d_bucket_d, d_dstart, d_flags, d_rtab;
    DBuf d_solid_removed;
    RoundStats round_stats[ROUND_KINDS] = {{GASM_MAX_TIP_ROUNDS}, {GASM_MAX_BUBBLE_ROUNDS}, {GASM_MAX_COV_ROUNDS}};
    DBuf d_ccov;
    std::vector<u64> h_ccov_m;
    std::vector<u32> h_ccov_n;
    bool coverage_queued = false;
    PassState links, pairs, map, mapg;
    PassState mapscore;
    int mapscore_shift[GASM_MAX_TABLES] = {};
    DBuf d_spectrum;
    DBuf d_twin;
    std::vector<u32> h_twin;
    bool fetched_twins = false;
    DBuf d_dk_key, d_dk_cnt, d_eflag, d_nxt, d_link, d_clen, d_ecid, d_ecoff;
    DBuf d_seg_cbases, d_seg_cstart, d_seg_bstart, d_c_off, d_contig_ascii;
    std::vector<u64> h_seg_doff, h_dk_key, h_c_off, h_seg_coff;
    std::vector<u32> h_dk_cnt, h_nxt;
    std::vector<u64> h_solid_before, h_solid_after, h_spectrum;
    bool spectrum_queued = false;
    std::vector<u8> h_eflag;
    std::vector<char> h_contigs;
    bool fetched_distinct = false, fetched_contigs = false;
    void release();
};

struct ScoreTable {
    DBuf d_prob, d_row, d_fix;
    std::vector<double> h_prob;
    std::vector<double> h_row_prob;
    double h_absmax = 0;
    bool h_finite = false;
    int fix_shift = -1;
    u32 n_table = 0;
    int fixed_shift(u64 max_terms) const;
    int set_fixed(gasm_ctx* ctx, int shift);
    int set(gasm_ctx* ctx, const char* bp_kmer, const u64* bp_off, u64 n_table, const double* bp_prob);
    int set_standard(gasm_ctx* ctx, const double* table69904);
    void release();
};

struct ScoreState {
    DBuf d_tbl_off, d_seed, d_gpos, d_poscnt, d_total, d_out_f64, d_out_i32, d_freq, d_pd_off, d_pd, d_seg_empty, d_fxsum, d_first, d_first_off;
    std::vector<u64> h_toff;
    u32 n_paths = 0, n_table = 0;
    u32 n_tables = 1;
    size_t stride = 1;
    const BuildState* graph = nullptr;
    bool want_freq = false, want_pd = false, launched = false;
    bool verify = false;
    std::vector<double> h_bp, h_nf, h_nl, h_freq, h_pd;
    std::vector<int32_t> h_breaks, h_len;
    std::vector<u64> h_pd_off;
    bool valid = false;
    void release();
};

int pipeline_build(gasm_ctx* ctx, DevReads& rd, BuildState& bs, const BuildOpts& o);
int pipeline_build_finish(gasm_ctx* ctx, DevReads& rd, BuildState& bs, bool* rebuilt);
int pipeline_build_finish_n(gasm_ctx* ctx, DevReads* rd, u32 n_segments, BuildState& bs, bool* rebuilt);
enum : u32 { GASM_RUNG_EXACT = 1, GASM_RUNG_TABLE = 2, GASM_RUNG_BBITS = 4, GASM_RUNG_MULTI = 8, GASM_RUNG_ALL = 15 };
bool build_next_config(u32 ovf, u32 rungs, int words, int bb_cap, bool& single_pass, bool& small_tbl, int& bbits, bool& multi_pass);
void pipeline_build_plan(const DevReads& rd, const BuildState& bs, int32_t* row);
int plan_build(gasm_ctx* ctx, DevReads& rd, int k, u64 hint, BuildState& bs);
void distinct_caps(BuildState& bs, u32 n_segments);
int launch_distinct(gasm_ctx* ctx, DevReads& rd, BuildState& bs);
int launch_graph(gasm_ctx* ctx, u32 n_segments, BuildState& bs);
int pipeline_fetch_distinct(gasm_ctx* ctx, DevReads& rd, BuildState& bs);
int pipeline_fetch_contigs(gasm_ctx* ctx, DevReads& rd, BuildState& bs);
int pipeline_fetch_solid_stats(gasm_ctx* ctx, DevReads& rd, BuildState& bs);
int pipeline_fetch_round_stats(gasm_ctx* ctx, DevReads& rd, BuildState& bs, u32 kind);
int pipeline_contig_coverage(gasm_ctx* ctx, DevReads& rd, BuildState& bs);
int pipeline_fetch_contig_coverage(gasm_ctx* ctx, DevReads& rd, BuildState& bs);
int pipeline_contig_links(gasm_ctx* ctx, DevReads& rd, BuildState& bs, u32 span_len);
int pipeline_fetch_contig_links(gasm_ctx* ctx, DevReads& rd, BuildState& bs);
int pipeline_place_pairs(gasm_ctx* ctx, DevReads& rd_build, DevReads& rd, BuildState& bs, u32 max_insert);
int pipeline_fetch_pair_places(gasm_ctx* ctx, DevReads& rd, BuildState& bs);
int pipeline_map_reads(gasm_ctx* ctx, DevReads& rd_build, DevReads& rd, BuildState& bs, bool gapped, u32 max_edits, u32 max_gap, u32 end_gap = 0, bool trace = false);
int pipeline_fetch_read_map(gasm_ctx* ctx, DevReads& rd, BuildState& bs, bool gapped);
int pipeline_score_mapped(gasm_ctx* ctx, DevReads& rd_build, DevReads& rd, BuildState& bs, bool gapped, int kmer, ScoreTable* const* tbs, u32 T, bool partial);
int pipeline_fetch_mapped_scores(gasm_ctx* ctx, DevReads& rd, BuildState& bs);
int pipeline_kmer_spectrum(gasm_ctx* ctx, DevReads& rd, BuildState& bs);
int pipeline_fetch_kmer_spectrum(gasm_ctx* ctx, DevReads& rd, BuildState& bs);
// ... 27 lines not shown
```

### genomeassembler_dev_amd/csrc/pipeline.hip

```cpp
#include <atomic>
#include <chrono>
#include <thread>
#include "pipeline.h"

#include <algorithm>
#include <cmath>

__global__ void k_set_u64(u64* p, u64 v) { *p = v; }

__global__ void k_add_empty_reads(PathSet ps, const u64* __restrict__ seg_empty, u32* __restrict__ poscnt, u32* __restrict__ total) {
    const u32 seg = blockIdx.y;
    const u32 p = ps.seg_path_off[seg] + blockIdx.x * GASM_WG + threadIdx.x;
    if (p >= ps.seg_path_off[seg + 1]) return;
    const u32 e = (u32)seg_empty[seg];
    if (!e) return;
    if (ps.p_off[p + 1] > ps.p_off[p]) poscnt[ps.p_off[p]] += e;
    else total[p] += e;
}

struct Knobs {
    int dedup_tbl = 0, scatter_wgs = 8, hist_wgs = 64, rank_rounds = 18, bbits_add = 0, ruler_shift = 0;
    bool rank_global = false, sync_build = false;
    Knobs() {
        if (const char* v = getenv("GASM_DEDUP_TBL")) dedup_tbl = atoi(v);
// ... 301 lines not shown
    GCHK(d_words.ensure((nw + 4) * 8));
    HIPCHK(hipMemsetAsync(d_words.p, 0, (nw + 4) * 8, ctx->stream));
    if (n && src.total_bases) {
        const u32 g = std::min(64u, next_pow2_u32((src.max_len + 31) / 32));
        const u32 grid = (u32)std::min<u64>((n * g + GASM_WG - 1) / GASM_WG, (u64)ctx->n_cu * 64);
        GLAUNCH(ctx, "k_reads_both_strands", k_reads_both_strands, dim3(std::max(1u, grid)), dim3(GASM_WG), 0, src.d_words.as<u64>(),
                src.fixed_len ? (const u64*)nullptr : src.d_read_off.as<u64>(), src.d_seg_read_off.as<u64>(), src.fixed_len, S, n, g,
                d_words.as<unsigned long long>());
    }
    GCHK(finish_upload(ctx));
    strands_of = src.upload_id;
    return GASM_OK;
}

ReadSet DevReads::view() const {
    ReadSet v;
    v.words = d_words.as<u64>();
    v.read_off = (fixed_len && !positioned) ? nullptr : d_read_off.as<u64>();
    v.seg_read_off = d_seg_read_off.as<u64>();
    v.seg_tile_start = d_seg_tile_start.as<u32>();
    v.tile_info = d_tile_info.as<uint4>();
    v.fixed_len = fixed_len;
    v.n_segments = n_segments;
    return v;
}

void DevReads::release() { d_words.release(); d_read_off.release(); d_seg_read_off.release(); d_seg_tile_start.release(); d_tile_info.release(); }

int DevPaths::upload_dirs(gasm_ctx* ctx) {
    GCHK(h2d(ctx, d_p_off, h_p_off.data(), h_p_off.size() * 8));
    GCHK(h2d(ctx, d_seg_path_off, h_seg_path_off.data(), h_seg_path_off.size() * 4));
    std::vector<u64>& sb = h_seg_base_off;
    sb.resize(n_segments + 1);
    for (u32 s = 0; s <= n_segments; ++s) sb[s] = h_p_off[h_seg_path_off[s]];
    GCHK(h2d(ctx, d_seg_base_off, sb.data(), sb.size() * 8));
    return GASM_OK;
}

int DevPaths::pack_from_device_ascii(gasm_ctx* ctx, const u8* d_ascii) {
    DBuf err;
    GCHK(err.ensure(8));
    HIPCHK(hipMemsetAsync(err.p, 0, 8, ctx->stream));
    int st = pack_ascii(ctx, d_ascii, total_bases, d_words, err.as<u32>());
    u32 herr = 0;
    if (st == GASM_OK && hipMemcpyAsync(&herr, err.p, 4, hipMemcpyDeviceToHost, ctx->stream) != hipSuccess) st = GASM_ERR_HIP;
    if (st == GASM_OK && hipStreamSynchronize(ctx->stream) != hipSuccess) st = GASM_ERR_HIP;
    err.release();
    if (st != GASM_OK) return st;
    if (herr) { gasm_set_error("paths contain a base outside upper-case ACGT"); return GASM_ERR_NON_ACGT; }
    return GASM_OK;
}

int DevPaths::upload_ascii(gasm_ctx* ctx, const char* data, const u64* off, u32 np) {
    n_segments = 1; n_paths = np;
    b_p_off = nullptr; b_seg_path_off = nullptr; b_seg_base_off = nullptr;
    h_p_off.resize((size_t)np + 1);
    for (u32 i = 0; i <= np; ++i) {
        if (i && off[i] < off[i - 1]) { gasm_set_error("path offsets not monotone"); return GASM_ERR_INVALID; }
        h_p_off[i] = off[i] - off[0];
    }
    total_bases = h_p_off[np];
    if (total_bases >= 0xFFFFFFF0ull) { gasm_set_error("paths exceed 2^32 bases"); return GASM_ERR_CAPACITY; }
    h_seg_path_off = {0u, np};
    DBuf ascii;
    GCHK(h2d(ctx, ascii, data + off[0], total_bases));
    int st = pack_from_device_ascii(ctx, ascii.as<u8>());
    ascii.release();
    GCHK(st);
    return upload_dirs(ctx);
}

PathSet DevPaths::view() const {
    PathSet v;
    v.words = d_words.as<u64>();
    v.p_off = b_p_off ? b_p_off : d_p_off.as<u64>();
    v.seg_path_off = b_seg_path_off ? b_seg_path_off : d_seg_path_off.as<u32>();
    v.n_segments = n_segments;
    return v;
}

void DevPaths::release() { d_words.release(); d_p_off.release(); d_seg_path_off.release(); d_seg_base_off.release(); }

void BuildState::release() {
    for (DBuf* b : {&d_solid_removed, &d_ccov, &links.d, &pairs.d, &map.d, &mapg.d, &mapscore.d, &d_spectrum, &d_twin, &d_keys, &d_keys2, &d_mult, &d_hist, &d_toff, &d_tcnt, &d_fdir, &d_bstart, &d_bucket_d, &d_dstart, &d_flags, &d_dk_key, &d_dk_cnt,
                    &d_eflag, &d_nxt, &d_link, &d_clen, &d_ecid, &d_ecoff, &d_rtab, &d_seg_cbases, &d_seg_cstart,
                    &d_seg_bstart, &d_c_off, &d_contig_ascii})
        b->release();
    for (RoundStats& rs : round_stats) rs.d_stats.release();
    part_valid = false;
    if (h_report) { (void)hipHostFree(h_report); h_report = nullptr; h_report_words = 0; }
}

void ScoreState::release() {
    for (DBuf* b : {&d_tbl_off, &d_seed, &d_gpos, &d_poscnt, &d_total, &d_out_f64, &d_out_i32, &d_freq, &d_pd_off, &d_pd, &d_seg_empty, &d_fxsum, &d_first, &d_first_off}) b->release();
}

static int ensure_lds_attrs(gasm_ctx* ctx) {
    if (ctx->lds_attrs_set) return GASM_OK;
#define GASM_LDS_ATTR(kern, bytes) HIPCHK(hipFuncSetAttribute(reinterpret_cast<const void*>(kern), hipFuncAttributeMaxDynamicSharedMemorySize, bytes));
#define GASM_SCORE_LDS_ATTR(T) GASM_LDS_ATTR((k_score_reads_graph<K, T>), GASM_SCORE_PATH_CAP * 12)
    for (int words = 1; words <= 2; ++words)
        GCHK(with_key(words, [&](auto tag) -> int {
            using K = typename decltype(tag)::type;
            GASM_LDS_ATTR(k_bucket_scatter<K>, 160 * 1024) GASM_LDS_ATTR(k_bucket_partition<K>, 160 * 1024) GASM_LDS_ATTR(k_tile_hist<K>, 160 * 1024)
            GASM_SCORE_LDS_ATTR(1) GASM_SCORE_LDS_ATTR(2) GASM_SCORE_LDS_ATTR(3) GASM_SCORE_LDS_ATTR(4) GASM_SCORE_LDS_ATTR(5) GASM_SCORE_LDS_ATTR(6) GASM_SCORE_LDS_ATTR(7) GASM_SCORE_LDS_ATTR(8)
            return GASM_OK;
        }));
    GASM_LDS_ATTR(k_rank_lds, 160 * 1024 - 64)
#define GASM_MAPSCORE_LDS_ATTR(T) GASM_LDS_ATTR((k_score_mapped<T, false>), GASM_SCORE_PATH_CAP * 12) GASM_LDS_ATTR((k_score_mapped<T, true>), GASM_SCORE_PATH_CAP * 12)
    GASM_MAPSCORE_LDS_ATTR(1) GASM_MAPSCORE_LDS_ATTR(2) GASM_MAPSCORE_LDS_ATTR(3) GASM_MAPSCORE_LDS_ATTR(4) GASM_MAPSCORE_LDS_ATTR(5) GASM_MAPSCORE_LDS_ATTR(6)
    GASM_MAPSCORE_LDS_ATTR(7) GASM_MAPSCORE_LDS_ATTR(8)
#undef GASM_MAPSCORE_LDS_ATTR
#undef GASM_SCORE_LDS_ATTR
#undef GASM_LDS_ATTR
    ctx->lds_attrs_set = true;
    return GASM_OK;
}

void distinct_caps(BuildState& bs, u32 S) {
    const u64 limit = bs.multi_pass ? GASM_BUCKET_MAX : bs.small_tbl ? GASM_TBL_LIMIT / 2 : GASM_TBL_LIMIT;
    const u64 per_seg = ((u64)1 << bs.bbits) * limit;
    const u64 all = bs.k < 16 ? ((u64)1 << (2 * bs.k)) : ~(u64)0;
    bs.D_cap = 0; bs.maxD_cap = 0;
    for (u32 s = 0; s < S; ++s) {
        const u64 c = std::min(std::min(bs.h_seg_nk[s], per_seg), all);
        bs.D_cap += c;
        bs.maxD_cap = std::max(bs.maxD_cap, c);
    }
}

static int launch_graph_dense(gasm_ctx* ctx, u32 S, BuildState& bs, bool last_pass);

static GraphView graph_view(const BuildState& bs) {
    GraphView gv;
    gv.dk_key = bs.d_dk_key.p;
    gv.dstart = bs.d_dstart.as<u32>();
    gv.fdir = bs.d_fdir.as<u16>();
    gv.k = bs.k;
    gv.bbits = bs.bbits;
    gv.fbits = bs.fbits;
    return gv;
}

static bool have_contigs(const BuildState& bs) { return bs.n_contigs && bs.d_total && bs.n_kmers; }

static ContigIndex contig_index(const BuildState& bs) {
    return ContigIndex{bs.d_link.as<u64>(), bs.d_ecid.as<u32>(), bs.d_c_off.as<u64>(), bs.d_seg_cstart.as<u32>(), bs.d_contig_ascii.as<u8>(), have_contigs(bs) ? 1 : 0};
}

template <class K, int TBL>
static int launch_bucket_dedup_as(gasm_ctx* ctx, BuildState& bs, u32 nbt, const u32* d_blen, u32* d_scan_out) {
    GLAUNCH(ctx, "k_bucket_dedup", (k_bucket_dedup<K, TBL>), dim3(nbt), dim3(GASM_WG), 0, bs.d_keys.as<K>(), bs.d_mult.as<u32>(), bs.d_bstart.as<u64>(), d_blen,
            bs.d_bucket_d.as<u32>(), bs.d_flags.as<u32>(), bs.d_fdir.as<u16>(), 2 * bs.k - bs.bbits, d_scan_out);
    return GASM_OK;
}
static int launch_bucket_dedup(gasm_ctx* ctx, BuildState& bs, u32 nbt, const u32* d_blen, u32* d_scan_out) {
    if (bs.words == 2) return launch_bucket_dedup_as<K128, 2048>(ctx, bs, nbt, d_blen, d_scan_out);
    if (bs.small_tbl) return launch_bucket_dedup_as<u64, 2048>(ctx, bs, nbt, d_blen, d_scan_out);
    return launch_bucket_dedup_as<u64, 4096>(ctx, bs, nbt, d_blen, d_scan_out);
}

int launch_distinct(gasm_ctx* ctx, DevReads& rd, BuildState& bs) {
    GasmRange range("gasm:distinct (partition + de-duplication)");
    const int k = bs.k, W = bs.words, bbits = bs.bbits;
    const size_t KB = 8 * (size_t)W;
    const u32 S = rd.n_segments, nb = 1u << bbits, nbt = S * nb;
    const u64 N = bs.n_kmers;
    const u32 line_keys = 128 / KB;
    const u32 pad_room = (u32)with_key(W, [](auto tag) -> int { return TileStage<typename decltype(tag)::type>::PAD_ROOM; });
    u32 padm = line_keys - 1;
    while (padm && (u64)nb * (padm + (W == 2 ? 1u : 0u)) > pad_room) padm >>= 1;
    const ReadSet rs = rd.view();
    const u32 g = bs.tile_g;
    const u32 grid_tiles = std::min<u32>(rd.n_tiles, (u32)ctx->n_cu * (u32)knobs().hist_wgs);
    const u32 scratch_keys = GASM_FLUSH_SLOTS * (16 / KB);
    GCHK(bs.d_bstart.ensure(((size_t)nbt + 1) * 8));
    GCHK(bs.d_bucket_d.ensure((size_t)nbt * 4));
    GCHK(bs.d_dstart.ensure(((size_t)nbt + 2) * 4));
    u64 n_alloc;
    const u32* d_blen = nullptr;
    const bool single = bs.single_pass && !bs.multi_pass && nb <= GASM_TILE_WG;
    bs.part_single = single;
    if (single) {
        const int slack = env_int("GASM_PART_SLACK", 100), forced = env_int("GASM_DBG_PART_CAP", 0);
        BuildState::PartLayout layout;
        layout.reads_id = rd.upload_id; layout.k = k; layout.bbits = bbits; layout.slack = slack; layout.forced = forced; layout.padm = padm; layout.g = g;
        if (!(bs.part_valid && bs.part == layout)) {
            std::vector<u64> h((size_t)nbt + 1);
            u64 at = 0;
            for (u32 s = 0; s < S; ++s) {
                const u64 mean = ceil_div_u64(bs.h_seg_nk[s], nb), tiles = rd.h_seg_tile_start[s + 1] - rd.h_seg_tile_start[s];
                u64 cap = mean + (u64)((double)mean * std::max(slack, 0) / 100.0) + (u64)(8.0 * std::sqrt((double)mean)) + 32 + tiles * padm;
                if (forced > 0) cap = (u64)forced;
                cap = (cap + line_keys - 1) / line_keys * line_keys;
                for (u32 b = 0; b < nb; ++b) { h[(size_t)s * nb + b] = at; at += cap; }
            }
            h[nbt] = at;
            bs.part_alloc = at;
            GCHK(h2d(ctx, bs.d_bstart, h.data(), h.size() * 8));
            HIPCHK(hipStreamSynchronize(ctx->stream));
            bs.part_valid = true;
            bs.part = layout;
        }
        n_alloc = bs.part_alloc;
        GCHK(bs.d_keys.ensure((n_alloc + scratch_keys) * KB));
        GCHK(bs.d_mult.ensure(n_alloc * 4));
        GCHK(bs.d_flags.ensure(GASM_FLAG_BYTES + (size_t)nbt * 4));
        HIPCHK(hipMemsetAsync(bs.d_flags.p, 0, GASM_FLAG_BYTES + (size_t)nbt * 4, ctx->stream));
        u32* const d_cursor = bs.d_flags.as<u32>() + GASM_FLAG_CURSORS;
        d_blen = d_cursor;
        u32 grid_part = std::min<u32>(rd.n_tiles, (u32)ctx->n_cu * (u32)knobs().scatter_wgs);
        if (const int cap = env_int("GASM_DBG_PART_GRID", 0)) grid_part = std::min<u32>(grid_part, (u32)std::max(1, cap));
        GLAUNCH_K(ctx, W, "k_bucket_partition", k_bucket_partition<K>, dim3(grid_part), dim3(GASM_TILE_WG), PartitionLds<K>{nb}.total(), rs, rs.tile_info, k, bbits, g, padm, rd.n_tiles,
                  bs.d_bstart.as<u64>(), d_cursor, bs.d_keys.as<K>(), n_alloc, bs.d_flags.as<u32>());
    } else {
        bs.part_valid = false;
        GCHK(bs.d_hist.ensure((size_t)nbt * 4));
        GCHK(bs.d_toff.ensure((size_t)rd.n_tiles * nb * 4));
        n_alloc = N + (u64)padm * rd.n_tiles * nb;
        GCHK(bs.d_keys.ensure((n_alloc + scratch_keys) * KB));
        GCHK(bs.d_mult.ensure(n_alloc * 4));
        GCHK(bs.d_tcnt.ensure((size_t)rd.n_tiles * nb * 8 + 64));
        GLAUNCH_K(ctx, W, "k_tile_hist", k_tile_hist<K>, dim3(grid_tiles), dim3(GASM_TILE_WG), (size_t)nb * 16, rs, rs.tile_info, k, bbits, g, rd.n_tiles,
                  bs.d_tcnt.as<ushort4>());
        GLAUNCH(ctx, "k_tile_scan", k_tile_scan, dim3(S, std::max(1u, nb / 32u)), dim3(1024), 0, rs, bbits, padm, bs.d_tcnt.as<ushort4>(),
                bs.d_toff.as<u32>(), bs.d_hist.as<u32>(), bs.d_flags.as<u32>());
        GLAUNCH(ctx, "k_scan_excl", k_scan_excl<u64>, dim3(1), dim3(1024), 0, bs.d_hist.as<u32>(), bs.d_bstart.as<u64>(), nbt);
        const u32 grid_scatter = std::min<u32>(rd.n_tiles, (u32)ctx->n_cu * (u32)knobs().scatter_wgs);
        GLAUNCH_K(ctx, W, "k_bucket_scatter", k_bucket_scatter<K>, dim3(grid_scatter), dim3(GASM_TILE_WG), ScatterLds<K>{nb}.total(), rs, rs.tile_info, k, bbits, g, padm, rd.n_tiles,
                  bs.d_bstart.as<u64>(), bs.d_toff.as<u32>(), bs.d_tcnt.as<ushort4>(), bs.d_keys.as<K>(), n_alloc);
    }
    const bool scan_in_dedup = !bs.multi_pass && nbt <= 16384 && env_int("GASM_SCAN_IN_DEDUP", 1) != 0;
    bs.scan_in_dedup = scan_in_dedup;
    u32* const d_scan_out = scan_in_dedup ? bs.d_dstart.as<u32>() : nullptr;
    bs.fbits = dedup_fbits(bs.small_tbl && !bs.multi_pass ? 2048 : GASM_TBL);
    GCHK(bs.d_fdir.ensure((size_t)nbt * ((1u << bs.fbits) + 1) * 2));
    if (bs.multi_pass) {
        GCHK(bs.d_keys2.ensure(n_alloc * KB));
        GLAUNCH_K(ctx, W, "k_bucket_dedup_multi", k_bucket_dedup_multi<K>, dim3(nbt), dim3(GASM_WG), 0, bs.d_keys.as<K>(), bs.d_keys2.as<K>(),
                  bs.d_mult.as<u32>(), bs.d_bstart.as<u64>(), bs.d_bucket_d.as<u32>(), bs.d_flags.as<u32>(), bs.d_fdir.as<u16>(), 2 * k - bbits);
        HIPCHK(hipMemcpyAsync(bs.d_keys.p, bs.d_keys2.p, n_alloc * KB, hipMemcpyDeviceToDevice, ctx->stream));
    } else {
        GCHK(launch_bucket_dedup(ctx, bs, nbt, d_blen, d_scan_out));
    }
    if (bs.opts.min_count > 1) {
        GCHK(bs.d_solid_removed.ensure((size_t)S * 4));
        HIPCHK(hipMemsetAsync(bs.d_solid_removed.p, 0, (size_t)S * 4, ctx->stream));
        GLAUNCH_K(ctx, W, "k_bucket_solid", k_bucket_solid<K>, dim3(nbt), dim3(GASM_WG), 0, bs.d_keys.as<K>(), bs.d_mult.as<u32>(), bs.d_bstart.as<u64>(),
                  bs.d_bucket_d.as<u32>(), bs.d_fdir.as<u16>(), 2 * k - bbits, bs.fbits, bbits, bs.opts.min_count, bs.d_solid_removed.as<u32>(),
                  bs.d_flags.as<u32>() + GASM_FLAG_SOLID_DONE, d_scan_out);
    }
    if (!scan_in_dedup) GLAUNCH(ctx, "k_scan_excl", k_scan_excl<u32>, dim3(1), dim3(1024), 0, bs.d_bucket_d.as<u32>(), bs.d_dstart.as<u32>(), nbt);
    return GASM_OK;
}

static int alloc_graph(BuildState& bs, u32 S) {
    const u64 D = std::max<u64>(bs.D_cap, 1);
    const size_t KB = 8 * (size_t)bs.words;
    if (D >= 0xFFFFFFF0ull) { gasm_set_error("more than 2^32 distinct k-mers possible in one batch: split it"); return GASM_ERR_CAPACITY; }
    GCHK(bs.d_dk_key.ensure(D * KB));
    GCHK(bs.d_dk_cnt.ensure(D * 4));
    GCHK(bs.d_eflag.ensure(D));
    GCHK(bs.d_nxt.ensure(D * 4));
    GCHK(bs.d_link.ensure(D * 8));
    GCHK(bs.d_clen.ensure(D * 4));
    GCHK(bs.d_ecid.ensure(D * 4));
    GCHK(bs.d_ecoff.ensure(D * 8));
    GCHK(bs.d_rtab.ensure((D / 2 + S + 2) * 4));
    GCHK(bs.d_seg_cbases.ensure((size_t)S * 8 + (size_t)S * 4));
    GCHK(bs.d_seg_cstart.ensure(((size_t)S + 1) * 4));
    GCHK(bs.d_seg_bstart.ensure(((size_t)S + 1) * 8));
    bs.bases_cap = D * (u64)bs.k;
    if (bs.bases_cap >= 0xFFFFFFF0ull) { gasm_set_error("contigs could exceed 2^32 bases: split the batch"); return GASM_ERR_CAPACITY; }
    GCHK(bs.d_c_off.ensure((D + 1) * 8));
    GCHK(bs.d_contig_ascii.ensure(bs.bases_cap + 64));
    return GASM_OK;
}

int launch_graph(gasm_ctx* ctx, u32 S, BuildState& bs) {
    const int W = bs.words, bbits = bs.bbits;
    const u32 nb = 1u << bbits, nbt = S * nb;
    GCHK(alloc_graph(bs, S));
    u32* const d_claim = bs.d_nxt.as<u32>();
    const BuildOpts& o = bs.opts;
    const u32 rounds = o.total_rounds();
    for (u32 kind = 0; kind < ROUND_KINDS; ++kind) {
        RoundStats& rs = bs.round_stats[kind];
        if (!o.rounds(kind)) continue;
        GCHK(rs.d_stats.ensure((size_t)2 * rs.max_rounds * S * 4));
        HIPCHK(hipMemsetAsync(rs.d_stats.p, 0, (size_t)2 * rs.max_rounds * S * 4, ctx->stream));
    }
    for (u32 r = 0; r <= rounds; ++r) {
        GLAUNCH_K(ctx, W, "k_bucket_gather", k_bucket_gather<K>, dim3(nbt), dim3(GASM_WG), 0, bs.d_keys.as<K>(), bs.d_mult.as<u32>(),
                  bs.d_bstart.as<u64>(), bs.d_dstart.as<u32>(), bs.d_dk_key.as<K>(), bs.d_dk_cnt.as<u32>(), d_claim, bs.d_eflag.as<u8>(), bs.d_flags.as<u32>());
        GCHK(launch_graph_dense(ctx, S, bs, r == rounds));
        if (r == rounds) break;
        u32 kind = ROUNDS_TIP, kr = r;
        while (kr >= o.rounds(kind)) kr -= o.rounds(kind++);
        static const char* const range_name[ROUND_KINDS] = {"gasm:tips (mark, compact)", "gasm:bubbles (mark, compact)", "gasm:lowcov (mark, compact)"};
        GasmRange range(range_name[kind]);
        const RoundStats& rs = bs.round_stats[kind];
        u32* const d_contigs = rs.d_stats.as<u32>() + (size_t)kr * S;
        u32* const d_kmers = rs.d_stats.as<u32>() + ((size_t)rs.max_rounds + kr) * S;
        const u32 est = std::max<u32>(1, (u32)std::min<u64>(bs.maxD_est, bs.maxD_cap));
        const u32 dchunks = (u32)ceil_div_u64(est, GASM_WG);
        if (kind == ROUNDS_TIP) {
            GLAUNCH_K(ctx, W, "k_tip_mark", k_tip_mark<K>, seg_grid(dchunks, S), dim3(GASM_WG), 0, graph_view(bs), S, dchunks, bs.d_eflag.as<u8>(), bs.d_clen.as<u32>(),
                      bs.d_nxt.as<u32>(), bs.d_dk_cnt.as<u32>(), bs.d_bstart.as<u64>(), bs.d_mult.as<u32>(), o.tip_len, bs.d_flags.as<u32>(), d_contigs);
        } else if (kind == ROUNDS_BUBBLE) {
            GLAUNCH_K(ctx, W, "k_bubble_mark", k_bubble_mark<K>, seg_grid(dchunks, S), dim3(GASM_WG), 0, graph_view(bs), S, dchunks, bs.d_eflag.as<u8>(),
                      bs.d_clen.as<u32>(), bs.d_nxt.as<u32>(), bs.d_dk_cnt.as<u32>(), bs.d_bstart.as<u64>(), bs.d_mult.as<u32>(), o.bubble_len,
                      bs.d_flags.as<u32>(), d_contigs);
        } else {
            GLAUNCH_K(ctx, W, "k_lowcov_mark", k_lowcov_mark<K>, seg_grid(dchunks, S), dim3(GASM_WG), 0, graph_view(bs), S, dchunks, bs.d_eflag.as<u8>(),
                      bs.d_clen.as<u32>(), bs.d_nxt.as<u32>(), bs.d_dk_cnt.as<u32>(), bs.d_bstart.as<u64>(), bs.d_mult.as<u32>(), o.cov_len, o.cov_cutoff,
                      bs.d_flags.as<u32>(), d_contigs);
        }
        u32* const d_scan_out = bs.scan_in_dedup ? bs.d_dstart.as<u32>() : nullptr;
        GLAUNCH_K(ctx, W, "k_bucket_solid", k_bucket_solid<K>, dim3(nbt), dim3(GASM_WG), 0, bs.d_keys.as<K>(), bs.d_mult.as<u32>(), bs.d_bstart.as<u64>(),
// ... 88 lines not shown
    u64 N = 0, maxNs = 0;
    bs.h_seg_nk.assign(S, 0);
    if (rd.fixed_len) {
        const u64 nk = rd.fixed_len >= (u32)k ? rd.fixed_len - k + 1 : 0;
        for (u32 s = 0; s < S; ++s) bs.h_seg_nk[s] = (rd.h_seg_read_off[s + 1] - rd.h_seg_read_off[s]) * nk;
    } else {
        u32 s = 0;
        for (u64 r = 0; r < rd.n_reads; ++r) {
            while (r >= rd.h_seg_read_off[s + 1]) ++s;
            const u64 L = rd.h_read_off[r + 1] - rd.h_read_off[r];
            if (L >= (u64)k) bs.h_seg_nk[s] += L - k + 1;
        }
    }
    for (u64 v : bs.h_seg_nk) { N += v; maxNs = std::max(maxNs, v); }
    bs.n_kmers = N;
    const u32 nk_max = rd.max_len >= (u32)k ? rd.max_len - k + 1 : 0;
    u32 g = next_pow2_u32((nk_max + KT - 1) / KT);
    g = std::max(1u, std::min((u32)GASM_TILE_WG, g));
    bs.tile_g = g;
    const u32 ipt = GASM_TILE_WG / g;
    const u32 orr = std::max(1u, (nk_max + g * KT - 1) / (g * KT));
    if (orr > 0xFFFFu) { gasm_set_error("reads longer than %u bases are not supported", GASM_TILE_WG * KT * 0xFFFFu); return GASM_ERR_CAPACITY; }
    bs.tile_orr = orr;
    GCHK(rd.set_tiles(ctx, ipt, orr));
    bs.bb_cap = std::min(10, 2 * (k - 1));
    const u64 dest = hint ? hint : std::max<u64>(1, maxNs / 8);
    if (!same || !bs.have_actual) {
        int bbits = 0;
        while (bbits < bs.bb_cap && (dest >> bbits) > 900) ++bbits;
        for (int extra = 0; extra < 2 && bbits < bs.bb_cap && ((u64)S << bbits) < 1024; ++extra) ++bbits;
        bbits = std::min(bs.bb_cap, bbits + knobs().bbits_add);
        bs.bbits = bbits;
        bs.small_tbl = (dest >> bbits) <= 900;
        if (knobs().dedup_tbl) bs.small_tbl = knobs().dedup_tbl == 2048;
        if (W == 2) bs.small_tbl = true;
        bs.maxD_est = (u32)std::min<u64>(dest, 0xFFFFFFF0ull);
        bs.have_actual = false;
        bs.rank_global = false;
        bs.multi_pass = false;
        bs.single_pass = env_int("GASM_SINGLE_PASS", 1) != 0;
    }
    GCHK(bs.d_flags.ensure(GASM_FLAG_BYTES));
    bs.d_total = 0; bs.n_contigs = 0; bs.contig_bases = 0;
    return GASM_OK;
}

static void zero_results(BuildState& bs, u32 S) {
    bs.h_dstart.assign((size_t)S + 1, 0);
    bs.h_seg_cstart.assign((size_t)S + 1, 0);
    bs.h_seg_bstart.assign((size_t)S + 1, 0);
    bs.d_total = 0; bs.n_contigs = 0; bs.contig_bases = 0;
}

int build_opts_check(const BuildOpts& o) {
    if (o.min_count < 1) { gasm_set_error("min_count must be >= 1 (1 keeps every k-mer)"); return GASM_ERR_INVALID; }
    if (o.strands != 1 && o.strands != 2) { gasm_set_error("strands must be 1 or 2 (got %u)", o.strands); return GASM_ERR_INVALID; }
    if (o.tip_len && (o.tip_rounds < 1 || o.tip_rounds > GASM_MAX_TIP_ROUNDS)) {
        gasm_set_error("tip_rounds must be 1..%d when tip_len > 0 (got %u)", GASM_MAX_TIP_ROUNDS, o.tip_rounds);
        return GASM_ERR_INVALID;
    }
    if (o.bubble_len > GASM_MAX_BUBBLE_LEN) { gasm_set_error("bubble_len must be <= %d (got %u)", GASM_MAX_BUBBLE_LEN, o.bubble_len); return GASM_ERR_INVALID; }
    if (o.bubble_len && (o.bubble_rounds < 1 || o.bubble_rounds > GASM_MAX_BUBBLE_ROUNDS)) {
        gasm_set_error("bubble_rounds must be 1..%d when bubble_len > 0 (got %u)", GASM_MAX_BUBBLE_ROUNDS, o.bubble_rounds);
        return GASM_ERR_INVALID;
    }
    if (o.cov_len > GASM_MAX_BUBBLE_LEN) { gasm_set_error("cov_len must be <= %d (got %u)", GASM_MAX_BUBBLE_LEN, o.cov_len); return GASM_ERR_INVALID; }
    if (o.lowcov() && (o.cov_rounds < 1 || o.cov_rounds > GASM_MAX_COV_ROUNDS)) {
        gasm_set_error("cov_rounds must be 1..%d when cov_cutoff > 0 and cov_len > 0 (got %u)", GASM_MAX_COV_ROUNDS, o.cov_rounds);
        return GASM_ERR_INVALID;
    }
    return GASM_OK;
}

BuildOpts build_opts_normalised(BuildOpts o) {
    if (!o.tip_len) o.tip_rounds = 0;
    if (!o.bubble_len) o.bubble_rounds = 0;
    if (!o.lowcov()) o.cov_rounds = 0;
    return o;
}

int pipeline_build(gasm_ctx* ctx, DevReads& rd, BuildState& bs, const BuildOpts& o) {
    if (o.strands == 2 && !rd.strands_of) { gasm_set_error("a both-strand build needs the both-strand reads"); return GASM_ERR_STATE; }
    GCHK(plan_build(ctx, rd, o.k, o.strands == 2 ? 2 * o.genome_len_hint : o.genome_len_hint, bs));
    bs.opts = build_opts_normalised(o);
    bs.fetched_twins = false;
    bs.spectrum_queued = false;
    bs.coverage_queued = false;
    for (PassState* ps : {&bs.links, &bs.pairs, &bs.map, &bs.mapg, &bs.mapscore}) ps->queued = false;
    const u32 S = rd.n_segments;
    zero_results(bs, S);
    bs.part_single = bs.scan_in_dedup = bs.ranked_in_lds = false;
    bs.ruler_shift = 0;
    bs.attempts_distinct = bs.n_kmers ? 1 : 0;
    bs.attempts_graph = 0;
    if (bs.n_kmers == 0) {
        bs.bbits = 0; bs.D_cap = 0; bs.maxD_cap = 0;
        GCHK(alloc_graph(bs, S));
        GCHK(bs.d_dstart.ensure(((size_t)S + 2) * 4));
        HIPCHK(hipMemsetAsync(bs.d_dstart.p, 0, ((size_t)S + 2) * 4, ctx->stream));
        HIPCHK(hipMemsetAsync(bs.d_seg_cstart.p, 0, ((size_t)S + 1) * 4, ctx->stream));
        HIPCHK(hipMemsetAsync(bs.d_seg_bstart.p, 0, ((size_t)S + 1) * 8, ctx->stream));
        HIPCHK(hipMemsetAsync(bs.d_c_off.p, 0, 8, ctx->stream));
        HIPCHK(hipStreamSynchronize(ctx->stream));
        return GASM_OK;
    }
    distinct_caps(bs, S);
    GCHK(launch_distinct(ctx, rd, bs));
    GCHK(launch_graph(ctx, S, bs));
    if (knobs().sync_build) GCHK(pipeline_build_finish(ctx, rd, bs, nullptr));
    return GASM_OK;
}

bool build_next_config(u32 ovf, u32 rungs, int words, int bb_cap, bool& single_pass, bool& small_tbl, int& bbits, bool& multi_pass) {
    if ((rungs & GASM_RUNG_EXACT) && (ovf & GASM_OVF_REGION) && single_pass) single_pass = false;
    else if ((rungs & GASM_RUNG_TABLE) && small_tbl && words == 1) small_tbl = false;
    else if ((rungs & GASM_RUNG_BBITS) && bbits < bb_cap) bbits = std::min(bb_cap, bbits + 2);
    else if ((rungs & GASM_RUNG_MULTI) && !multi_pass) multi_pass = true;
    else return false;
    return true;
}

int pipeline_build_finish(gasm_ctx* ctx, DevReads& rd, BuildState& bs, bool* rebuilt) {
    return pipeline_build_finish_n(ctx, &rd, rd.n_segments, bs, rebuilt);
}

int pipeline_build_finish_n(gasm_ctx* ctx, DevReads* rd, u32 S, BuildState& bs, bool* rebuilt) {
    if (rebuilt) *rebuilt = false;
    if (!bs.pending) return GASM_OK;
    HIPCHK(hipSetDevice(ctx->device));
    for (;;) {
        const BuildReport<const u32> rep{bs.h_report, S};
        GCHK(wait_report(ctx, &rep.ticket(), bs.ticket));
        bs.pending = false;
        const u32 overflow = rep.flags() & (GASM_OVF_TABLE | GASM_OVF_REGION);
        if (!overflow && !rep.rank_failed() && !(rep.flags() & GASM_OVF_TIP_RANK)) break;
        if (rebuilt) *rebuilt = true;
        if (overflow) {
            if (!rd) { gasm_set_error("a merged k-mer bucket overflowed its table: the pooled build needs more bucket bits"); return GASM_ERR_CAPACITY; }
            if (!build_next_config(overflow, GASM_RUNG_ALL, bs.words, bs.bb_cap, bs.single_pass, bs.small_tbl, bs.bbits, bs.multi_pass)) {
                gasm_set_error("a k-mer bucket holds more than %d distinct k-mers even with %d bucket bits", GASM_BUCKET_MAX, bs.bbits);
                return GASM_ERR_CAPACITY;
            }
            distinct_caps(bs, S);
            ++bs.attempts_distinct;
            GCHK(launch_distinct(ctx, *rd, bs));
        } else {
            bs.rank_global = true;
            ++bs.attempts_graph;
            if (bs.opts.total_rounds() && rd) { ++bs.attempts_distinct; GCHK(launch_distinct(ctx, *rd, bs)); }
        }
        GCHK(launch_graph(ctx, S, bs));
    }
    const BuildReport<const u32> rep{bs.h_report, S};
    bs.h_dstart.assign(&rep.dstart(0), &rep.dstart(S) + 1);
    u32 maxD = 0;
    for (u32 s = 0; s <= S; ++s) {
        bs.h_seg_cstart[s] = rep.cstart(s);
        bs.h_seg_bstart[s] = (u64)rep.bstart_lo(s) | ((u64)rep.bstart_hi(s) << 32);
        if (s < S) maxD = std::max(maxD, rep.dstart(s + 1) - rep.dstart(s));
    }
    bs.d_total = bs.h_dstart[S];
    bs.n_contigs = bs.h_seg_cstart[S];
    bs.contig_bases = bs.h_seg_bstart[S];
    bs.maxD_est = std::max(1u, maxD);
    bs.paths_est = 1;
    for (u32 s = 0; s < S; ++s) bs.paths_est = std::max(bs.paths_est, bs.h_seg_cstart[s + 1] - bs.h_seg_cstart[s]);
    bs.have_actual = true;
    return GASM_OK;
}

void pipeline_build_plan(const DevReads& rd, const BuildState& bs, int32_t* row) {
    row[GASM_PLAN_KEY_WORDS] = bs.words;
    row[GASM_PLAN_BUCKET_BITS] = bs.bbits;
    row[GASM_PLAN_TABLE_SLOTS] = bs.small_tbl ? 2048 : 4096;
    row[GASM_PLAN_SINGLE_PASS] = bs.part_single;
    row[GASM_PLAN_MULTI_PASS] = bs.multi_pass;
    row[GASM_PLAN_SCAN_IN_DEDUP] = bs.scan_in_dedup;
    row[GASM_PLAN_RANKED_IN_LDS] = bs.ranked_in_lds;
    row[GASM_PLAN_RULER_SHIFT] = (int32_t)bs.ruler_shift;
    row[GASM_PLAN_RANK_GLOBAL] = bs.rank_global || knobs().rank_global;
    row[GASM_PLAN_TILE_G] = (int32_t)bs.tile_g;
    row[GASM_PLAN_OFFSET_ROUNDS] = (int32_t)bs.tile_orr;
    row[GASM_PLAN_DISTINCT_ATTEMPTS] = (int32_t)bs.attempts_distinct;
    row[GASM_PLAN_GRAPH_ATTEMPTS] = (int32_t)bs.attempts_graph;
    row[GASM_PLAN_K] = bs.k;
    row[GASM_PLAN_SEGMENTS] = (int32_t)rd.n_segments;
}

int pipeline_fetch_distinct(gasm_ctx* ctx, DevReads& rd, BuildState& bs) {
    GCHK(pipeline_build_finish(ctx, rd, bs, nullptr));
    if (bs.fetched_distinct) return GASM_OK;
    const u32 S = rd.n_segments;
    bs.h_seg_doff.resize((size_t)S + 1);
    for (u32 s = 0; s <= S; ++s) bs.h_seg_doff[s] = bs.h_dstart.empty() ? 0 : bs.h_dstart[s];
    bs.h_dk_key.resize((size_t)bs.d_total * bs.words);
    bs.h_dk_cnt.resize(bs.d_total);
    if (bs.d_total) {
        HIPCHK(hipMemcpyAsync(bs.h_dk_key.data(), bs.d_dk_key.p, (size_t)bs.d_total * 8 * bs.words, hipMemcpyDeviceToHost, ctx->stream));
        HIPCHK(hipMemcpyAsync(bs.h_dk_cnt.data(), bs.d_dk_cnt.p, (size_t)bs.d_total * 4, hipMemcpyDeviceToHost, ctx->stream));
    }
    HIPCHK(hipStreamSynchronize(ctx->stream));
    bs.fetched_distinct = true;
    return GASM_OK;
}

int pipeline_fetch_round_stats(gasm_ctx* ctx, DevReads& rd, BuildState& bs, u32 kind) {
    GCHK(pipeline_build_finish(ctx, rd, bs, nullptr));
    RoundStats& rs = bs.round_stats[kind];
    const u32 S = rd.n_segments, R = rs.max_rounds;
    rs.h_contigs.assign((size_t)S * R, 0); rs.h_kmers.assign((size_t)S * R, 0);
    if (!bs.opts.rounds(kind) || !bs.n_kmers) return GASM_OK;
    std::vector<u32> h((size_t)2 * R * S);
    GCHK(d2h_sync(ctx, h.data(), rs.d_stats.p, h.size() * 4));
    for (u32 s = 0; s < S; ++s)
        for (u32 r = 0; r < R; ++r) { rs.h_contigs[(size_t)s * R + r] = h[(size_t)r * S + s]; rs.h_kmers[(size_t)s * R + r] = h[((size_t)R + r) * S + s]; }
    return GASM_OK;
}

int pipeline_fetch_solid_stats(gasm_ctx* ctx, DevReads& rd, BuildState& bs) {
    GCHK(pipeline_build_finish(ctx, rd, bs, nullptr));
    const u32 S = rd.n_segments;
    std::vector<u32> removed(S, 0);
    if (bs.opts.min_count > 1 && bs.n_kmers) GCHK(d2h_sync(ctx, removed.data(), bs.d_solid_removed.p, (size_t)S * 4));
    bs.h_solid_before.resize(S); bs.h_solid_after.resize(S);
    for (u32 kind = 0; kind < ROUND_KINDS; ++kind) if (bs.opts.rounds(kind)) GCHK(pipeline_fetch_round_stats(ctx, rd, bs, kind));
    for (u32 s = 0; s < S; ++s) {
        bs.h_solid_after[s] = bs.h_dstart.empty() ? 0 : bs.h_dstart[s + 1] - bs.h_dstart[s];
        for (u32 kind = 0; kind < ROUND_KINDS; ++kind) {
            const RoundStats& rs = bs.round_stats[kind];
            if (bs.opts.rounds(kind)) for (u32 r = 0; r < rs.max_rounds; ++r) bs.h_solid_after[s] += rs.h_kmers[(size_t)s * rs.max_rounds + r];
        }
        bs.h_solid_before[s] = bs.h_solid_after[s] + removed[s];
    }
    return GASM_OK;
}

int pipeline_kmer_spectrum(gasm_ctx* ctx, DevReads& rd, BuildState& bs) {
    GCHK(pipeline_build_finish(ctx, rd, bs, nullptr));
    HIPCHK(hipSetDevice(ctx->device));
    const u32 S = rd.n_segments;
    GCHK(bs.d_spectrum.ensure((size_t)S * 256 * 4));
    HIPCHK(hipMemsetAsync(bs.d_spectrum.p, 0, (size_t)S * 256 * 4, ctx->stream));
    if (bs.d_total) {
// ... 886 lines not shown
```

### include/gasm.h

```cpp
#ifndef GASM_H
#define GASM_H

#include <stdint.h>

#ifdef __cplusplus
extern "C" {
#endif

typedef enum gasm_status {
    GASM_OK = 0,
    GASM_ERR_INVALID = -1,
    GASM_ERR_NON_ACGT = -2,
    GASM_ERR_NO_DEVICE = -3,
    GASM_ERR_HIP = -4,
    GASM_ERR_CAPACITY = -5,
    GASM_ERR_RANGE = -6,
    GASM_ERR_STATE = -7,
    GASM_ERR_INTERNAL = -8
} gasm_status;

#define GASM_MAX_K 63
#define GASM_TABLE_ROWS 69904

typedef struct gasm_ctx gasm_ctx;
// ... 206 lines not shown
                              const uint32_t** mult, int* words);
int gasm_batch_fetch_graph(gasm_batch* b, const uint8_t** edge_flags, const uint32_t** edge_next);
int gasm_batch_fetch_contigs(gasm_batch* b, const uint64_t** seg_contig_off , const uint64_t** off,
                             const char** data);
int gasm_batch_fetch_scores(gasm_batch* b, const double** bp_score, const double** norm_by_break_freqs,
                            const double** norm_by_len, const int32_t** kmer_breaks, const int32_t** sequence_len);

int gasm_batch_count_read_kmers(gasm_batch* b);
int gasm_batch_fetch_read_kmer_counts(gasm_batch* b, const uint32_t** counts);
int gasm_count_read_kmers(gasm_ctx* ctx, const char* reads, const uint64_t* read_off, uint64_t n_reads, int kmer, const char* keys,
                          const uint64_t* key_off, uint64_t n_keys, uint32_t* counts);

typedef struct gasm_pool gasm_pool;
int gasm_pool_create(gasm_ctx* ctx, const char* reads, uint64_t n_reads, uint32_t fixed_len, const uint64_t* seg_read_off,
                     uint32_t n_segments, gasm_pool** out);
void gasm_pool_free(gasm_pool* p);
int gasm_pool_key_words(const gasm_pool* p);
int gasm_pool_local_runs(gasm_pool* p, int k, int bbits, const uint32_t** run_len);
int gasm_pool_pack_runs(gasm_pool* p, const uint32_t* bucket_ix, uint64_t n, void* d_keys_out, void* d_counts_out);
int gasm_pool_merge_runs(gasm_pool* p, uint32_t n_out, uint32_t n_src, const uint64_t* run_off, const uint32_t* run_len,
                         const void* d_keys_in, const void* d_counts_in, const uint32_t** merged_len);
int gasm_pool_fetch_fine_directory(gasm_pool* p, const uint16_t** fdir, int* fbits);
int gasm_pool_graph(gasm_pool* p, uint32_t n_local_segments);
int gasm_pool_piece_words(gasm_pool* p, uint32_t seg_lo, uint32_t seg_hi, uint64_t* n_words );
int gasm_pool_pack_reads(gasm_pool* p, uint32_t seg_lo, uint32_t seg_hi, void* d_words_out);
int gasm_pool_set_reads(gasm_pool* p, const void* d_words, uint64_t n_words, uint32_t n_pieces, const uint32_t* piece_seg,
                        const uint64_t* piece_reads, const uint64_t* piece_word_off);
int gasm_pool_score(gasm_pool* p, int kmer, const double* table);
int gasm_pool_fetch_distinct(gasm_pool* p, const uint64_t** seg_off, const uint64_t** keys, const uint32_t** mult, int* words);
int gasm_pool_fetch_contigs(gasm_pool* p, const uint64_t** seg_contig_off, const uint64_t** off, const char** data);
int gasm_pool_fetch_scores(gasm_pool* p, const double** bp_score, const double** norm_by_break_freqs, const double** norm_by_len,
                           const int32_t** kmer_breaks, const int32_t** sequence_len);

#define GASM_COMM_ID_BYTES 128
typedef struct gasm_comm gasm_comm;
int gasm_comm_unique_id(void* id );
int gasm_comm_create(gasm_ctx* ctx, const void* id, int rank, int world, gasm_comm** out);
int gasm_comm_create_virtual(gasm_ctx* ctx, int world, gasm_comm** out);
void gasm_comm_destroy(gasm_comm* c);
int gasm_comm_world(const gasm_comm* c);
int gasm_comm_rank(const gasm_comm* c);
int gasm_comm_stage(const gasm_comm* c);
int gasm_comm_keep_plans(gasm_comm* c, int on);
int gasm_comm_fetch_plan(gasm_comm* c, int which, uint32_t local_rank, uint64_t* sizes , const uint64_t** send_off,
                         const uint64_t** send_tot, const uint64_t** run_off, const uint32_t** run_len, const uint64_t** recv_tot,
                         const uint64_t** bstart, const uint64_t** info );
int gasm_pool_bucket_owner(uint32_t n_segments, int bbits, uint32_t world, uint32_t* owner );
int gasm_pool_segment_bounds(uint32_t n_segments, uint32_t world, uint32_t* first );
int gasm_pool_exchange_build(gasm_comm* c, gasm_pool* const* pools, uint32_t n_pools, int k, int bbits, int kmer,
                             const double* table , uint64_t* stats );

int gasm_batch_guided(gasm_batch* b);
int gasm_batch_fetch_guided(gasm_batch* b, const uint64_t** seg_off , const uint64_t** off, const char** data,
                            const double** bp_score, const double** norm_by_len, const int32_t** kmer_breaks);
int gasm_batch_fetch_score_fixed(gasm_batch* b, const int64_t** fx, int* shift);

int gasm_batch_score_tables(gasm_batch* b, int kmer, const double* tables, uint32_t n_tables);
int gasm_batch_fetch_scores_table(gasm_batch* b, uint32_t t, const double** bp_score, const double** norm_by_break_freqs,
                                  const double** norm_by_len, const int32_t** kmer_breaks, const int32_t** sequence_len);
int gasm_batch_fetch_score_fixed_table(gasm_batch* b, uint32_t t, const int64_t** fx, int* shift);

int gasm_profile_enable(gasm_ctx* ctx, int on);
int gasm_profile_filter(gasm_ctx* ctx, const char* names);
int gasm_profile_reset(gasm_ctx* ctx);
int gasm_profile_read(gasm_ctx* ctx, int* n, const char* const** names, const double** ms, const uint64_t** launches);

#define GASM_PLAN_FIELDS 15
#define GASM_PLAN_KEY_WORDS 0
#define GASM_PLAN_BUCKET_BITS 1
#define GASM_PLAN_TABLE_SLOTS 2
#define GASM_PLAN_SINGLE_PASS 3
#define GASM_PLAN_MULTI_PASS 4
#define GASM_PLAN_SCAN_IN_DEDUP 5
#define GASM_PLAN_RANKED_IN_LDS 6
#define GASM_PLAN_RULER_SHIFT 7
#define GASM_PLAN_RANK_GLOBAL 8
#define GASM_PLAN_TILE_G 9
#define GASM_PLAN_OFFSET_ROUNDS 10
#define GASM_PLAN_DISTINCT_ATTEMPTS 11
#define GASM_PLAN_GRAPH_ATTEMPTS 12
#define GASM_PLAN_K 13
#define GASM_PLAN_SEGMENTS 14
int gasm_batch_build_plan(gasm_batch* b, int32_t* out, int n);

#ifdef __cplusplus
}
#endif
#endif
```

Before: 234.4 billion k-mers/s.

## Partition paired (k+1)-mer records and merge them into k-mer counts

Adds a pair mode to the single-pass bucket partition. It emits one (k+1)-mer record for every second k-mer position instead of one record per k-mer, which roughly halves the keys scattered and deduplicated. A new k_pair_merge kernel then splits the deduplicated (k+1)-mers into their prefix and suffix k-mers. It gathers these from the matching sub-buckets and inserts them into the final per-bucket hash table with weighted counts. The mode is enabled by default for large read sets with even k-mer counts per read and falls back to the normal build on overflow, at the cost of an extra kernel launch, extra buffers and a more complex cross-bucket gather.

After: 276.7 billion k-mers/s (median of 6 runs). 1.18x the previous value.

```diff
diff --git a/genomeassembler_dev_amd/_lib.py b/genomeassembler_dev_amd/_lib.py
--- a/genomeassembler_dev_amd/_lib.py
+++ b/genomeassembler_dev_amd/_lib.py
@@ -125,6 +125,7 @@
     "gasm_batch_fetch_guided": (_int, [_vp, _PP, _PP, _PP, _PP, _PP, _PP]),
     "gasm_batch_fetch_score_fixed": (_int, [_vp, _PP, C.POINTER(_int)]),
     "gasm_batch_build_plan": (_int, [_vp, C.POINTER(_i32), _int]),
+    "gasm_batch_build_pair_records": (_int, [_vp]),
     "gasm_batch_simulate": (_int, [_vp, _vp, _vp, _u32, _u32, C.c_double, _u64, _int, _vp, _PP]),
     "gasm_batch_fetch_read_starts": (_int, [_vp, _PP, _PP]),
     "gasm_read_files": (_int, [_vp, _u32, _int, _PP]),
diff --git a/genomeassembler_dev_amd/batch.py b/genomeassembler_dev_amd/batch.py
--- a/genomeassembler_dev_amd/batch.py
+++ b/genomeassembler_dev_amd/batch.py
@@ -339,6 +339,18 @@
         blocks = [dict(zip(PLAN_FIELDS, out[j * len(PLAN_FIELDS):(j + 1) * len(PLAN_FIELDS)])) for j in range(rows)]
         return dict(blocks[0], blocks=blocks)
 
+    def build_pair_records(self):
+        r = lib().gasm_batch_build_pair_records(self.h)
+        if r < 0:
+            check(r)
+        return r == 1
+
+    def build_pair_fell_back(self):
+        r = lib().gasm_batch_build_pair_records(self.h)
+        if r < 0:
+            check(r)
+        return r == 2
+
     def score(self, kmer=8, table=None):
         t = np.ascontiguousarray(qtable.load_normalised() if table is None else table, dtype=np.float64)
         if t.size != qtable.ROWS:
diff --git a/genomeassembler_dev_amd/csrc/capi.hip b/genomeassembler_dev_amd/csrc/capi.hip
--- a/genomeassembler_dev_amd/csrc/capi.hip
+++ b/genomeassembler_dev_amd/csrc/capi.hip
@@ -1272,6 +1272,15 @@
     API_GUARD_END
 }
 
+int gasm_batch_build_pair_records(gasm_batch* b) {
+    API_GUARD_BEGIN
+    if (!b) { gasm_set_error("gasm_batch_build_pair_records: bad argument"); return GASM_ERR_INVALID; }
+    if (!b->built) { gasm_set_error("gasm_batch_build_pair_records before gasm_batch_build"); return GASM_ERR_STATE; }
+    GCHK(batch_finish(b));
+    return b->S().bs.pair_ran ? 1 : b->S().bs.pair_fell_back ? 2 : 0;
+    API_GUARD_END
+}
+
 int gasm_batch_count_read_kmers(gasm_batch* b) {
     API_GUARD_BEGIN
     if (!b) { gasm_set_error("batch is null"); return GASM_ERR_INVALID; }
diff --git a/genomeassembler_dev_amd/csrc/kernels.h b/genomeassembler_dev_amd/csrc/kernels.h
--- a/genomeassembler_dev_amd/csrc/kernels.h
+++ b/genomeassembler_dev_amd/csrc/kernels.h
@@ -89,6 +89,7 @@
     GASM_OVF_TABLE = 1,
     GASM_OVF_REGION = 2,
     GASM_OVF_TIP_RANK = 4,
+    GASM_REP_PAIR = 8,
 };
 static_assert(GASM_FLAG_ACTIVE + GASM_FLAG_ACTIVE_N <= GASM_FLAG_WORDS && GASM_FLAG_WORDS * 4 == GASM_FLAG_BYTES, "flag area layout");
 
@@ -145,9 +146,15 @@
 __global__ void k_bucket_scatter(ReadSet rs, const uint4* tinfo, int k, int bbits, u32 g, u32 padm, u32 n_tiles, const u64* bstart, const u32* toff,
                                  const ushort4* tcnt, K* keys, u64 scratch);
 #define GASM_RT_MAX 16
-template <class K>
+#define GASM_PAIR_NFL 6
+#define GASM_PAIR_MAX_BUCKETS 256
+#define GASM_PAIR_MIN_KMERS (8ull << 20)
+template <class K, bool PAIR = false>
 __global__ void k_bucket_partition(ReadSet rs, const uint4* tinfo, int k, int bbits, u32 g, u32 padm, u32 n_tiles, const u64* bstart, u32* cursor,
                                    K* keys, u64 scratch, u32* flags);
+template <class K, int TBL>
+__global__ void k_pair_merge(const K* ykeys, const u32* ycnt, const u16* yfdir, const u64* ybstart, K* keys, u32* mult, const u64* bstart, u32* bucket_d, u32* overflow,
+                             u16* fdir, int k, int bbits, u32* dstart);
 template <class K, int TBL>
 __global__ void k_bucket_dedup(K* keys, u32* mult, const u64* bstart, const u32* blen, u32* bucket_d, u32* overflow, u16* fdir, int low_bits, u32* dstart);
 #define GASM_BUCKET_MAX 65535
diff --git a/genomeassembler_dev_amd/csrc/kernels_build.hip b/genomeassembler_dev_amd/csrc/kernels_build.hip
--- a/genomeassembler_dev_amd/csrc/kernels_build.hip
+++ b/genomeassembler_dev_amd/csrc/kernels_build.hip
@@ -337,15 +337,18 @@
 template __global__ void k_bucket_scatter<u64>(ReadSet, const uint4*, int, int, u32, u32, u32, const u64*, const u32*, const ushort4*, u64*, u64);
 template __global__ void k_bucket_scatter<K128>(ReadSet, const uint4*, int, int, u32, u32, u32, const u64*, const u32*, const ushort4*, K128*, u64);
 
-template <class K>
+template <class K, bool PAIR>
 __global__ void __launch_bounds__(GASM_TILE_WG, 4) k_bucket_partition(ReadSet rs, const uint4* __restrict__ tinfo, int k, int bbits, u32 g, u32 padm,
                                                                     u32 n_tiles, const u64* __restrict__ bstart, u32* __restrict__ cursor,
                                                                     K* __restrict__ keys, u64 scratch, u32* __restrict__ flags) {
     extern __shared__ __align__(16) unsigned char s_raw[];
     constexpr u32 KT = KeyTraits<K>::KT;
-    constexpr u32 NFL = KeyTraits<K>::NFL;
+    constexpr u32 STEP = PAIR ? 2 : 1;
+    constexpr u32 NK = KT / STEP;
+    constexpr u32 NFL = PAIR ? GASM_PAIR_NFL : KeyTraits<K>::NFL;
     constexpr u32 KPU = TileStage<K>::KPU;
-    constexpr u32 CAP = TileStage<K>::CAP;
+    constexpr u32 CAP = NFL * GASM_TILE_WG * KPU;
+    static_assert(!PAIR || (sizeof(K) == 8 && (CAP + TileStage<K>::TRASH) * 8 + (CAP + TileStage<K>::TRASH) / 2 <= TileStage<K>::BYTES), "the bucket bytes lie in the staging area's spare part");
     const u32 nb = 1u << bbits;
     const u32 tid = threadIdx.x, wv = tid >> 6, ln = tid & 63, sub = tid & 3u;
     const PartitionLds<K> lds{nb};
@@ -355,7 +358,10 @@
     u32* s_cnt = s_base + lds.n_sub() + lds.n_dummy;
     u32* s_tmp = s_cnt + lds.n_sub() + lds.n_dummy;
     u32* s_cin = s_tmp + lds.n_tmp;
+    u8* s_bk = reinterpret_cast<u8*>(s_key + CAP + TileStage<K>::TRASH);
     const int bshift = 2 * k - bbits;
+    const int pshift = bbits + 62 - 2 * k;
+    auto filler = [&](u32 b) { if constexpr (PAIR) return (K)(1ull << 63); else return key_filler<K>(b, bshift); };
     const bool carry = padm != 0;
     const u32 ush = carry ? (u32)__builtin_ctz(padm + 1) - (KPU == 2 ? 1u : 0u) : 0u;
     const u32 n_carry = carry ? nb << ush : 0u;
@@ -380,11 +386,11 @@
         const auto w = rl.prep();
         const u32 nv_now = nv;
         const u32 seg = ti.seg;
-        u32 idx[KT];
-        static_for<KT>([&](auto J) {
-            constexpr u32 j = J;
+        u32 idx[NK];
+        static_for<NK>([&](auto J) {
+            constexpr u32 j = J * STEP;
             const u32 bkt = bbits ? w.template top_hi<j>() >> (32 - bbits) : 0u;
-            idx[j] = atomicAdd(&s_cnt[j < nv_now ? 4 * bkt + sub : 4 * nb], 1u);
+            idx[J] = atomicAdd(&s_cnt[j < nv_now ? 4 * bkt + sub : 4 * nb], 1u);
         });
         const u32 tnext = tile + 1 < tile_end ? tile + 1 : tile;
         const TileInfo tin = tile_decode(tinfo, tnext);
@@ -429,24 +435,32 @@
                 } else {
                     if (f < n) *reinterpret_cast<u64x2*>(dst) = cu;
                 }
+                if constexpr (PAIR) if (f < n) s_bk[((v >> 5) + f) >> 1] = (u8)b;
             }
             const u32 v = s_comb[b].w, n = v & 31u;
             if ((v >> 31) && n) {
                 K* const dst = s_key + ((v << 1) >> 6) + f;
-                if (f >= n) dst[0] = key_filler<K>(b, bshift);
-                if constexpr (KPU == 2) if (f + 1 >= n) dst[1] = key_filler<K>(b, bshift);
+                if (f >= n) dst[0] = filler(b);
+                if constexpr (KPU == 2) if (f + 1 >= n) dst[1] = filler(b);
+                if constexpr (PAIR) s_bk[(((v << 1) >> 6) + f) >> 1] = (u8)b;
             }
         }
         {
-            static_for<KT>([&](auto J) {
-                constexpr u32 j = J;
+            static_for<NK>([&](auto J) {
+                constexpr u32 j = J * STEP;
                 const u32 bkt = bbits ? w.template top_hi<j>() >> (32 - bbits) : 0u;
-                idx[j] += s_base[4 * bkt + sub];
+                idx[J] += s_base[4 * bkt + sub];
             });
             const u32 trash = CAP + wv * 8 + (ln & 7u);
-            static_for<KT>([&](auto J) {
-                constexpr u32 j = J;
-                s_key[j < nv_now ? idx[j] : trash] = w.template key<j>(k);
+            static_for<NK>([&](auto J) {
+                constexpr u32 j = J * STEP;
+                if constexpr (PAIR) {
+                    const u32 slot = j < nv_now ? idx[J] : trash;
+                    s_key[slot] = (w.template top<j>() << bbits) >> pshift;
+                    s_bk[slot >> 1] = (u8)(w.template top_hi<j>() >> (32 - bbits));
+                } else {
+                    s_key[j < nv_now ? idx[J] : trash] = w.template key<j>(k);
+                }
             });
         }
         if (t < nb) {
@@ -464,7 +478,7 @@
             if (last && n && !(c.z >> 31)) {
                 u64x2 o = cu;
                 if constexpr (KPU == 2) {
-                    const u64 fl = key_filler<u64>(b, bshift);
+                    const u64 fl = filler(b);
                     if (f >= n) o.x = fl;
                     if (f + 1 >= n) o.y = fl;
                 } else if (f >= n) {
@@ -485,7 +499,8 @@
 #pragma unroll
             for (u32 u = 0; u < 3; ++u) {
                 u32 bkt = 0;
-                if (bbits) {
+                if constexpr (PAIR) bkt = s_bk[t + GASM_TILE_WG * (u0 + u)] & (nb - 1);
+                else if (bbits) {
                     if constexpr (KPU == 2) bkt = (u32)(wd[u].x >> bshift) & (nb - 1);
                     else bkt = kfield(K128{wd[u].x, wd[u].y}, bshift) & (nb - 1);
                 }
@@ -503,8 +518,9 @@
         rl.template wait_all_but<NFL>();
     }
 }
-template __global__ void k_bucket_partition<u64>(ReadSet, const uint4*, int, int, u32, u32, u32, const u64*, u32*, u64*, u64, u32*);
-template __global__ void k_bucket_partition<K128>(ReadSet, const uint4*, int, int, u32, u32, u32, const u64*, u32*, K128*, u64, u32*);
+template __global__ void k_bucket_partition<u64, false>(ReadSet, const uint4*, int, int, u32, u32, u32, const u64*, u32*, u64*, u64, u32*);
+template __global__ void k_bucket_partition<u64, true>(ReadSet, const uint4*, int, int, u32, u32, u32, const u64*, u32*, u64*, u64, u32*);
+template __global__ void k_bucket_partition<K128, false>(ReadSet, const uint4*, int, int, u32, u32, u32, const u64*, u32*, K128*, u64, u32*);
 
 #define GASM_SLOT_LOCKED 0xFFFFFFFFu
 
@@ -518,7 +534,7 @@
 }
 
 template <int TBL>
-__device__ __forceinline__ bool dedup_step(u64* t_key, u32* t_cnt, u32* n_distinct, u64 key, u32& set) {
+__device__ __forceinline__ bool dedup_step(u64* t_key, u32* t_cnt, u32* n_distinct, u64 key, u32& set, u32 w = 1u) {
     constexpr u32 NSETS = TBL / 2;
     const u64x2 c = lds_load128(&t_key[2 * set]);
     int slot = c.x == key ? 0 : c.y == key ? 1 : -1;
@@ -531,7 +547,7 @@
         else if (old != key) return false;
         slot = emp;
     }
-    atomicAdd(&t_cnt[2 * set + slot], 1u);
+    atomicAdd(&t_cnt[2 * set + slot], w);
     return true;
 }
 template <int TBL>
@@ -734,6 +750,66 @@
 template __global__ void k_bucket_dedup<u64, 4096>(u64*, u32*, const u64*, const u32*, u32*, u32*, u16*, int, u32*);
 template __global__ void k_bucket_dedup<u64, 2048>(u64*, u32*, const u64*, const u32*, u32*, u32*, u16*, int, u32*);
 template __global__ void k_bucket_dedup<K128, 2048>(K128*, u32*, const u64*, const u32*, u32*, u32*, u16*, int, u32*);
+
+template <class K, int TBL>
+__global__ void __launch_bounds__(GASM_WG, TBL == 4096 ? 3 : GASM_DEDUP_WGS)
+k_pair_merge(const K* __restrict__ ykeys, const u32* __restrict__ ycnt, const u16* __restrict__ yfdir, const u64* __restrict__ ybstart, K* __restrict__ keys, u32* __restrict__ mult,
+             const u64* __restrict__ bstart, u32* __restrict__ bucket_d, u32* __restrict__ overflow, u16* __restrict__ fdir, int k, int bbits,
+             u32* __restrict__ dstart) {
+    static_assert(sizeof(K) == 8, "pair records are 64-bit keys");
+    constexpr int LIMIT = TBL / 16 * 11;
+    constexpr int BINS = dedup_bins(TBL);
+    constexpr int LOG_TBL = TBL == 4096 ? 12 : 11;
+    constexpr int LOG_SETS = LOG_TBL - 1;
+    constexpr u32 NSETS = 1u << LOG_SETS;
+    __shared__ __align__(32) K t_key[TBL];
+    __shared__ __align__(16) u32 t_cnt[TBL];
+    __shared__ u32 s_tmp[8];
+    u32* const s_start = reinterpret_cast<u32*>(t_key + LIMIT);
+    u32* const s_cur = s_start + BINS;
+    const u32 gb = blockIdx.x, nb = 1u << bbits, b = gb & (nb - 1), seg0 = gb - b;
+    if (gb == 0 && threadIdx.x == 0) atomicOr(overflow + GASM_FLAG_OVERFLOW, GASM_REP_PAIR);
+    for (u32 i = threadIdx.x; i < TBL; i += GASM_WG) { t_key[i] = key_empty<K>(); t_cnt[i] = 0; }
+    if (threadIdx.x == 0) { s_tmp[4] = 0; s_tmp[5] = 0; s_tmp[6] = 0; }
+    __syncthreads();
+    const int low = 2 * k - bbits;
+    const int ybins = low + 2 < LOG_TBL - 2 ? low + 2 : LOG_TBL - 2;
+    const u64 pre = (u64)b << low;
+    auto insert = [&](u64 key, u32 c) {
+        u32 st = khash(key) >> (32 - LOG_SETS);
+        bool ok = false;
+        for (u32 probe = 0; probe < 8 * NSETS && !ok; ++probe) ok = dedup_step<TBL>(t_key, t_cnt, &s_tmp[4], key, st, c);
+        if (!ok) s_tmp[5] = 1;
+    };
+    for (u32 l = 0; l < 5; ++l) {
+        const u32 src = l == 0 ? gb : seg0 + (((l - 1) << (bbits - 2)) | (b >> 2));
+        const u16* const row = yfdir + (u64)src * (BINS + 1);
+        const u32 lo = l == 0 ? 0u : row[(b & 3u) << (ybins - 2)];
+        const u32 hi = l == 0 ? row[BINS] : row[((b & 3u) + 1u) << (ybins - 2)];
+        const u64 at = ybstart[src];
+        for (u32 i = lo + threadIdx.x; i < hi; i += GASM_WG) {
+            if (__hip_atomic_load(&s_tmp[4], __ATOMIC_RELAXED, __HIP_MEMORY_SCOPE_WORKGROUP) > (u32)LIMIT) { s_tmp[5] = 1; break; }
+            const u64 y = ykeys[at + i];
+            insert(pre | (l == 0 ? y >> 2 : klowbits(y, low)), ycnt[at + i]);
+        }
+    }
+    __syncthreads();
+    const u64 beg = bstart[gb], room = bstart[gb + 1] - beg;
+    const bool no_table = s_tmp[5] || s_tmp[4] > (u32)LIMIT;
+    if (no_table || s_tmp[4] > room) {
+        for (u32 i = threadIdx.x; i <= (u32)BINS; i += GASM_WG) fdir[(u64)gb * (BINS + 1) + i] = 0;
+        if (threadIdx.x == 0) { atomicOr(overflow + GASM_FLAG_OVERFLOW, no_table ? GASM_OVF_TABLE : GASM_OVF_REGION); publish_u32(&bucket_d[gb], 0u); }
+        dedup_last_scan(bucket_d, dstart, gridDim.x, overflow + GASM_FLAG_DEDUP_DONE, s_tmp + 7, s_tmp);
+        return;
+    }
+    const u32 d = s_tmp[4];
+    dedup_order<K, TBL, true>(t_key, t_cnt, s_start, s_cur, s_tmp, fdir, gb, low, d);
+    for (u32 i = threadIdx.x; i < d; i += GASM_WG) { keys[beg + i] = t_key[i]; mult[beg + i] = t_cnt[i]; }
+    if (threadIdx.x == 0) publish_u32(&bucket_d[gb], d);
+    dedup_last_scan(bucket_d, dstart, gridDim.x, overflow + GASM_FLAG_DEDUP_DONE, s_tmp + 7, s_tmp);
+}
+template __global__ void k_pair_merge<u64, 4096>(const u64*, const u32*, const u16*, const u64*, u64*, u32*, const u64*, u32*, u32*, u16*, int, int, u32*);
+template __global__ void k_pair_merge<u64, 2048>(const u64*, const u32*, const u16*, const u64*, u64*, u32*, const u64*, u32*, u32*, u16*, int, int, u32*);
 
 template <class K>
 __global__ void __launch_bounds__(GASM_WG) k_bucket_dedup_multi(const K* __restrict__ keys, K* __restrict__ keys_out, u32* __restrict__ mult,
diff --git a/genomeassembler_dev_amd/csrc/pipeline.h b/genomeassembler_dev_amd/csrc/pipeline.h
--- a/genomeassembler_dev_amd/csrc/pipeline.h
+++ b/genomeassembler_dev_amd/csrc/pipeline.h
@@ -124,8 +124,9 @@
         u64 reads_id = 0;
         int k = 0, bbits = 0, slack = 0, forced = 0;
         u32 padm = 0, g = 0;
+        bool pair = false;
         bool operator==(const PartLayout& o) const {
-            return reads_id == o.reads_id && k == o.k && bbits == o.bbits && slack == o.slack && forced == o.forced && padm == o.padm && g == o.g;
+            return pair == o.pair && reads_id == o.reads_id && k == o.k && bbits == o.bbits && slack == o.slack && forced == o.forced && padm == o.padm && g == o.g;
         }
     } part;
     bool part_valid = false;
@@ -141,6 +142,11 @@
     bool have_actual = false;
     u32 tile_orr = 1;
     bool part_single = false;
+    bool pair_try = false;
+    bool pair_failed = false;
+    bool part_pair = false;
+    bool pair_ran = false;
+    bool pair_fell_back = false;
     bool scan_in_dedup = false;
     u32 ruler_shift = 0;
     u32 attempts_distinct = 0;
@@ -155,6 +161,9 @@
     std::vector<u32> h_seg_cstart;
     std::vector<u64> h_seg_bstart;
     DBuf d_keys2;
+    DBuf d_bstart2;
+    u64 part_alloc2 = 0;
+    DBuf d_mult2, d_fdir2;
     DBuf d_keys, d_mult, d_hist, d_toff, d_tcnt, d_fdir, d_bstart, d_bucket_d, d_dstart, d_flags, d_rtab;
     DBuf d_solid_removed;
     RoundStats round_stats[ROUND_KINDS] = {{GASM_MAX_TIP_ROUNDS}, {GASM_MAX_BUBBLE_ROUNDS}, {GASM_MAX_COV_ROUNDS}};
diff --git a/genomeassembler_dev_amd/csrc/pipeline.hip b/genomeassembler_dev_amd/csrc/pipeline.hip
--- a/genomeassembler_dev_amd/csrc/pipeline.hip
+++ b/genomeassembler_dev_amd/csrc/pipeline.hip
@@ -407,7 +407,7 @@
 void DevPaths::release() { d_words.release(); d_p_off.release(); d_seg_path_off.release(); d_seg_base_off.release(); }
 
 void BuildState::release() {
-    for (DBuf* b : {&d_solid_removed, &d_ccov, &links.d, &pairs.d, &map.d, &mapg.d, &mapscore.d, &d_spectrum, &d_twin, &d_keys, &d_keys2, &d_mult, &d_hist, &d_toff, &d_tcnt, &d_fdir, &d_bstart, &d_bucket_d, &d_dstart, &d_flags, &d_dk_key, &d_dk_cnt,
+    for (DBuf* b : {&d_solid_removed, &d_ccov, &links.d, &pairs.d, &map.d, &mapg.d, &mapscore.d, &d_spectrum, &d_twin, &d_keys, &d_keys2, &d_mult2, &d_fdir2, &d_bstart2, &d_mult, &d_hist, &d_toff, &d_tcnt, &d_fdir, &d_bstart, &d_bucket_d, &d_dstart, &d_flags, &d_dk_key, &d_dk_cnt,
                     &d_eflag, &d_nxt, &d_link, &d_clen, &d_ecid, &d_ecoff, &d_rtab, &d_seg_cbases, &d_seg_cstart,
                     &d_seg_bstart, &d_c_off, &d_contig_ascii})
         b->release();
@@ -428,6 +428,7 @@
         GCHK(with_key(words, [&](auto tag) -> int {
             using K = typename decltype(tag)::type;
             GASM_LDS_ATTR(k_bucket_scatter<K>, 160 * 1024) GASM_LDS_ATTR(k_bucket_partition<K>, 160 * 1024) GASM_LDS_ATTR(k_tile_hist<K>, 160 * 1024)
+            if constexpr (sizeof(K) == 8) GASM_LDS_ATTR((k_bucket_partition<K, true>), 160 * 1024)
             GASM_SCORE_LDS_ATTR(1) GASM_SCORE_LDS_ATTR(2) GASM_SCORE_LDS_ATTR(3) GASM_SCORE_LDS_ATTR(4) GASM_SCORE_LDS_ATTR(5) GASM_SCORE_LDS_ATTR(6) GASM_SCORE_LDS_ATTR(7) GASM_SCORE_LDS_ATTR(8)
             return GASM_OK;
         }));
@@ -475,6 +476,15 @@
 
 template <class K, int TBL>
 static int launch_bucket_dedup_as(gasm_ctx* ctx, BuildState& bs, u32 nbt, const u32* d_blen, u32* d_scan_out) {
+    if constexpr (sizeof(K) == 8) {
+        if (bs.part_pair) {
+            GLAUNCH(ctx, "k_bucket_dedup", (k_bucket_dedup<K, TBL>), dim3(nbt), dim3(GASM_WG), 0, bs.d_keys2.as<K>(), bs.d_mult2.as<u32>(), bs.d_bstart2.as<u64>(), d_blen,
+                    bs.d_bucket_d.as<u32>(), bs.d_flags.as<u32>(), bs.d_fdir2.as<u16>(), 2 * bs.k + 2 - bs.bbits, (u32*)nullptr);
+            GLAUNCH(ctx, "k_pair_merge", (k_pair_merge<K, TBL>), dim3(nbt), dim3(GASM_WG), 0, bs.d_keys2.as<K>(), bs.d_mult2.as<u32>(), bs.d_fdir2.as<u16>(), bs.d_bstart2.as<u64>(), bs.d_keys.as<K>(),
+                    bs.d_mult.as<u32>(), bs.d_bstart.as<u64>(), bs.d_bucket_d.as<u32>(), bs.d_flags.as<u32>(), bs.d_fdir.as<u16>(), bs.k, bs.bbits, d_scan_out);
+            return GASM_OK;
+        }
+    }
     GLAUNCH(ctx, "k_bucket_dedup", (k_bucket_dedup<K, TBL>), dim3(nbt), dim3(GASM_WG), 0, bs.d_keys.as<K>(), bs.d_mult.as<u32>(), bs.d_bstart.as<u64>(), d_blen,
             bs.d_bucket_d.as<u32>(), bs.d_flags.as<u32>(), bs.d_fdir.as<u16>(), 2 * bs.k - bs.bbits, d_scan_out);
     return GASM_OK;
@@ -506,23 +516,31 @@
     const u32* d_blen = nullptr;
     const bool single = bs.single_pass && !bs.multi_pass && nb <= GASM_TILE_WG;
     bs.part_single = single;
+    const bool pair = single && bs.pair_try && W == 1 && !rd.positioned && rd.fixed_len > (u32)k && ((rd.fixed_len - (u32)k + 1) & 1u) == 0 && bbits >= 2 &&
+                      nb <= GASM_PAIR_MAX_BUCKETS;
+    bs.part_pair = pair;
     if (single) {
         const int slack = env_int("GASM_PART_SLACK", 100), forced = env_int("GASM_DBG_PART_CAP", 0);
         BuildState::PartLayout layout;
-        layout.reads_id = rd.upload_id; layout.k = k; layout.bbits = bbits; layout.slack = slack; layout.forced = forced; layout.padm = padm; layout.g = g;
+        layout.reads_id = rd.upload_id; layout.k = k; layout.bbits = bbits; layout.slack = slack; layout.forced = forced; layout.padm = padm; layout.g = g; layout.pair = pair;
         if (!(bs.part_valid && bs.part == layout)) {
-            std::vector<u64> h((size_t)nbt + 1);
-            u64 at = 0;
+            std::vector<u64> h((size_t)nbt + 1), h2((size_t)nbt + 1);
+            u64 at = 0, at2 = 0;
             for (u32 s = 0; s < S; ++s) {
-                const u64 mean = ceil_div_u64(bs.h_seg_nk[s], nb), tiles = rd.h_seg_tile_start[s + 1] - rd.h_seg_tile_start[s];
-                u64 cap = mean + (u64)((double)mean * std::max(slack, 0) / 100.0) + (u64)(8.0 * std::sqrt((double)mean)) + 32 + tiles * padm;
-                if (forced > 0) cap = (u64)forced;
-                cap = (cap + line_keys - 1) / line_keys * line_keys;
-                for (u32 b = 0; b < nb; ++b) { h[(size_t)s * nb + b] = at; at += cap; }
+                const u64 tiles = rd.h_seg_tile_start[s + 1] - rd.h_seg_tile_start[s];
+                auto capacity = [&](u64 mean, u64 forced_cap) {
+                    u64 cap = mean + (u64)((double)mean * std::max(slack, 0) / 100.0) + (u64)(8.0 * std::sqrt((double)mean)) + 32 + tiles * padm;
+                    if (forced > 0) cap = forced_cap;
+                    return (cap + line_keys - 1) / line_keys * line_keys;
+                };
+                const u64 cap = capacity(ceil_div_u64(bs.h_seg_nk[s], nb), (u64)forced);
+                const u64 cap2 = capacity(ceil_div_u64(ceil_div_u64(bs.h_seg_nk[s], 2), nb), ((u64)std::max(forced, 0) + 1) / 2);
+                for (u32 b = 0; b < nb; ++b) { h[(size_t)s * nb + b] = at; at += cap; h2[(size_t)s * nb + b] = at2; at2 += cap2; }
             }
-            h[nbt] = at;
-            bs.part_alloc = at;
+            h[nbt] = at; h2[nbt] = at2;
+            bs.part_alloc = at; bs.part_alloc2 = at2;
             GCHK(h2d(ctx, bs.d_bstart, h.data(), h.size() * 8));
+            if (pair) GCHK(h2d(ctx, bs.d_bstart2, h2.data(), h2.size() * 8));
             HIPCHK(hipStreamSynchronize(ctx->stream));
             bs.part_valid = true;
             bs.part = layout;
@@ -536,6 +554,12 @@
         d_blen = d_cursor;
         u32 grid_part = std::min<u32>(rd.n_tiles, (u32)ctx->n_cu * (u32)knobs().scatter_wgs);
         if (const int cap = env_int("GASM_DBG_PART_GRID", 0)) grid_part = std::min<u32>(grid_part, (u32)std::max(1, cap));
+        if (pair) {
+            GCHK(bs.d_keys2.ensure((bs.part_alloc2 + scratch_keys) * KB));
+            GCHK(bs.d_mult2.ensure(bs.part_alloc2 * 4));
+            GLAUNCH(ctx, "k_bucket_partition", (k_bucket_partition<u64, true>), dim3(grid_part), dim3(GASM_TILE_WG), PartitionLds<u64>{nb}.total(), rs, rs.tile_info, k, bbits, g, padm,
+                    rd.n_tiles, bs.d_bstart2.as<u64>(), d_cursor, bs.d_keys2.as<u64>(), bs.part_alloc2, bs.d_flags.as<u32>());
+        } else
         GLAUNCH_K(ctx, W, "k_bucket_partition", k_bucket_partition<K>, dim3(grid_part), dim3(GASM_TILE_WG), PartitionLds<K>{nb}.total(), rs, rs.tile_info, k, bbits, g, padm, rd.n_tiles,
                   bs.d_bstart.as<u64>(), d_cursor, bs.d_keys.as<K>(), n_alloc, bs.d_flags.as<u32>());
     } else {
@@ -560,6 +584,7 @@
     u32* const d_scan_out = scan_in_dedup ? bs.d_dstart.as<u32>() : nullptr;
     bs.fbits = dedup_fbits(bs.small_tbl && !bs.multi_pass ? 2048 : GASM_TBL);
     GCHK(bs.d_fdir.ensure((size_t)nbt * ((1u << bs.fbits) + 1) * 2));
+    if (pair) GCHK(bs.d_fdir2.ensure((size_t)nbt * ((1u << bs.fbits) + 1) * 2));
     if (bs.multi_pass) {
         GCHK(bs.d_keys2.ensure(n_alloc * KB));
         GLAUNCH_K(ctx, W, "k_bucket_dedup_multi", k_bucket_dedup_multi<K>, dim3(nbt), dim3(GASM_WG), 0, bs.d_keys.as<K>(), bs.d_keys2.as<K>(),
@@ -814,6 +839,10 @@
 int pipeline_build(gasm_ctx* ctx, DevReads& rd, BuildState& bs, const BuildOpts& o) {
     if (o.strands == 2 && !rd.strands_of) { gasm_set_error("a both-strand build needs the both-strand reads"); return GASM_ERR_STATE; }
     GCHK(plan_build(ctx, rd, o.k, o.strands == 2 ? 2 * o.genome_len_hint : o.genome_len_hint, bs));
+    if (!bs.have_actual) bs.pair_failed = false;
+    const int pair_env = env_int("GASM_PAIR", -1);
+    bs.pair_try = !bs.pair_failed && (pair_env > 0 || (pair_env < 0 && bs.n_kmers >= GASM_PAIR_MIN_KMERS));
+    bs.pair_ran = bs.pair_fell_back = false;
     bs.opts = build_opts_normalised(o);
     bs.fetched_twins = false;
     bs.spectrum_queued = false;
@@ -869,6 +898,7 @@
         if (rebuilt) *rebuilt = true;
         if (overflow) {
             if (!rd) { gasm_set_error("a merged k-mer bucket overflowed its table: the pooled build needs more bucket bits"); return GASM_ERR_CAPACITY; }
+            if (bs.part_pair) bs.pair_try = false, bs.pair_failed = bs.pair_fell_back = true;
             if (!build_next_config(overflow, GASM_RUNG_ALL, bs.words, bs.bb_cap, bs.single_pass, bs.small_tbl, bs.bbits, bs.multi_pass)) {
                 gasm_set_error("a k-mer bucket holds more than %d distinct k-mers even with %d bucket bits", GASM_BUCKET_MAX, bs.bbits);
                 return GASM_ERR_CAPACITY;
@@ -891,6 +921,7 @@
         bs.h_seg_bstart[s] = (u64)rep.bstart_lo(s) | ((u64)rep.bstart_hi(s) << 32);
         if (s < S) maxD = std::max(maxD, rep.dstart(s + 1) - rep.dstart(s));
     }
+    bs.pair_ran = (rep.flags() & GASM_REP_PAIR) != 0;
     bs.d_total = bs.h_dstart[S];
     bs.n_contigs = bs.h_seg_cstart[S];
     bs.contig_bases = bs.h_seg_bstart[S];
diff --git a/include/gasm.h b/include/gasm.h
--- a/include/gasm.h
+++ b/include/gasm.h
@@ -312,6 +312,7 @@
 #define GASM_PLAN_K 13
 #define GASM_PLAN_SEGMENTS 14
 int gasm_batch_build_plan(gasm_batch* b, int32_t* out, int n);
+int gasm_batch_build_pair_records(gasm_batch* b);
 
 #ifdef __cplusplus
 }
```
